# pytorch/audio

Hardware: NVIDIA H100
Metric: MelSpectrogram frames/sec (higher is better)
Workload: dtype f32

## Files before the change

audio_b200/csrc/frontend_pow2.cu:

```cuda
#include <type_traits>
#include <utility>

#include "common.cuh"
#include "f32x2.cuh"
#include "ptx.cuh"

namespace b200a {

namespace {

constexpr float kKaldiEps = 1.1920928955078125e-07f;
constexpr int kPadSymmetric = 4;
constexpr int kWarps = 8;
constexpr int kMelWarps = 4;
constexpr int kMaxItems = 64;
constexpr int kMaxItemsPerWarp = 32;
constexpr int kFragSmemSteps = 112;
constexpr int kMaxSlots = 64;

template <int G>
struct Geo {
  static constexpr int kNfft = 32 * G;
  static constexpr int kBins = kNfft / 2 + 1;
  static constexpr int kGroups = 32 / G;
  static constexpr int kFrames = 2 * kGroups;
  static constexpr int kRowLd = G + 1;
  static constexpr int kRegion = 32 * (G + 1) + (G == 8 ? 8 : 0);
  static constexpr int kTileF2 = kGroups * kRegion;
  static constexpr int kSlots = kWarps * kFrames;
  static constexpr int kPitch = ((kBins + 7 - 4 + 31) / 32) * 32 + 4;
  static constexpr int kLogG = G == 32 ? 5 : (G == 16 ? 4 : 3);
};

struct MelItem {
  int tile;
  int kstart;
  int nsteps;
  int frag_off;
};
struct MelPlan {
  int n_tiles, n_items, total_steps, pad;
  int warp_cnt[kWarps];
  int warp_items[kWarps][kMaxItemsPerWarp];
  MelItem items[kMaxItems];
};

struct Pow2Extra {
  size_t tw2d, tw_eo, plan, frags, total;
};

inline int mel_tiles(int n_mels) { return (n_mels + 7) / 8; }

inline Pow2Extra pow2_layout(const b200a_frontend_desc& d, size_t base) {
  Pow2Extra e{};
  const size_t n_bins = d.n_fft / 2 + 1;
  const size_t nt = d.n_mels > 0 ? mel_tiles(d.n_mels) : 0;
  size_t off = base;
  e.tw2d = off;
  off = align_up(off + sizeof(float2) * 32 * 32, 256);
  e.tw_eo = off;
  off = align_up(off + sizeof(float2) * 17 * 32, 256);
  e.plan = off;
  off = align_up(off + sizeof(MelPlan), 256);
  e.frags = off;
  off = align_up(off + sizeof(float4) * 32 * nt * ((n_bins + 7) / 8 + 1), 256);
  e.total = off;
  return e;
}

bool pow2_applicable(const b200a_frontend_desc& d) {
  return (d.n_fft == 2048 || d.n_fft == 1024 || d.n_fft == 512 || d.n_fft == 256) && d.onesided != 0;
}

template <int... Is, typename F>
__device__ __forceinline__ void static_for_impl(std::integer_sequence<int, Is...>, F&& f) {
  (f(std::integral_constant<int, Is>{}), ...);
}
template <int N, typename F>
__device__ __forceinline__ void static_for(F&& f) {
  static_for_impl(std::make_integer_sequence<int, N>{}, static_cast<F&&>(f));
}

__host__ __device__ constexpr int brev5(int v) {
  return ((v & 1) << 4) | ((v & 2) << 2) | (v & 4) | ((v & 8) >> 2) | ((v & 16) >> 4);
}
template <int LOG>
__host__ __device__ constexpr int brev(int v) {
  return brev5(v) >> (5 - LOG);
}

__device__ constexpr float kCos32[17] = {1.f, 0.98078528040323043f, 0.92387953251128674f, 0.83146961230254524f,
                                         0.70710678118654757f, 0.55557023301960229f, 0.38268343236508984f,
                                         0.19509032201612833f, 0.f, -0.19509032201612819f, -0.38268343236508973f,
                                         -0.55557023301960196f, -0.70710678118654746f, -0.83146961230254535f,
                                         -0.92387953251128674f, -0.98078528040323043f, -1.f};
__device__ constexpr float kSin32[17] = {0.f, 0.19509032201612825f, 0.38268343236508978f, 0.55557023301960218f,
                                         0.70710678118654746f, 0.83146961230254524f, 0.92387953251128674f,
                                         0.98078528040323043f, 1.f, 0.98078528040323043f, 0.92387953251128674f,
                                         0.83146961230254546f, 0.70710678118654757f, 0.55557023301960218f,
                                         0.38268343236508989f, 0.19509032201612861f, 0.f};

template <int E>
__device__ __forceinline__ void bfly(float2& a, float2& b) {
  if constexpr (E == 0) {
    const float2 t = b;
    b = sub2(a, t);
    a = add2(a, t);
  } else if constexpr (E == 8) {
    const float2 t = b;
    b = add_i(a, t);
    a = sub_i(a, t);
  } else if constexpr (E == 4) {
    constexpr float c = 0.70710678118654752f;
    const float2 t = sub_i(b, b);
    b = fmas2(-c, t, a);
    a = fmas2(c, t, a);
  } else if constexpr (E == 12) {
    constexpr float c = 0.70710678118654752f;
    const float2 u = add_i(b, b);
    b = fmas2(c, u, a);
    a = fmas2(-c, u, a);
  } else {
    constexpr float wr = kCos32[E], wi = -kSin32[E];
    const float2 p = cfma2(wr, wi, b, a);
    b = fma2(make_float2(2.f, 2.f), a, make_float2(-p.x, -p.y));
    a = p;
  }
}

template <int LEN, int OFF, int S0 = 0, int S1 = 5>
__device__ __forceinline__ void fft_regs(float2 (&a)[32]) {
  constexpr int kStages = LEN == 32 ? 5 : (LEN == 16 ? 4 : 3);
  constexpr int kFirst = S0, kLast = S1 < kStages ? S1 : kStages;
  static_for<kLast - kFirst>([&](auto si) {
    constexpr int len = 2 << (decltype(si)::value + kFirst);
    constexpr int half = len / 2;
    static_for<LEN / 2>([&](auto bi) {
      constexpr int b = decltype(bi)::value;
      constexpr int i = (b / half) * len, j = b % half;
      bfly<j*(32 / len)>(a[OFF + i + j], a[OFF + i + j + half]);
    });
  });
}

struct Pow2Params {
  const float* wave;
  int64_t length, row_stride, frames, units_per_row, total_units;
  float* out;
  float* group_max;
  int64_t rows_per_group;
  const float* window;
  const float2* tw2d;
  const MelPlan* plan;
  const float4* frags;
  const WsHeader* hdr;
  int hop, pad, center, pad_mode, n_mels;
  int stage, log_mels, bulk_ok, stage_ok;
  int out_width, out_col0, out_vec;
  int kaldi, k_off, k_win, k_dc, k_energy_mode, k_energy_col, k_log;
  float k_preemph, k_energy_floor;
  float power, db_mult, db_amin, db_offset;
};

__device__ __forceinline__ int frame_lead(const Pow2Params& p, int n_fft) {
  return p.kaldi ? p.k_off : (p.center ? n_fft / 2 : 0);
}

constexpr int kComplexOut = 3;

template <int POWER_MODE>
__device__ __forceinline__ float pow_of(float re, float im, float power) {
  if constexpr (POWER_MODE == 2) return fmaf(re, re, im * im);
  const float mag = hypotf(re, im);
  return power == 1.f ? mag : powf(mag, power);
}

struct GroupMax {
  float* dst;
  int64_t group;
  float value;
  __device__ __forceinline__ void flush() {
    if (dst == nullptr) return;
    const int64_t g0 = __shfl_sync(0xffffffffu, group, 0);
    if (__all_sync(0xffffffffu, group == g0)) {
      const float mx = warp_max(value);
      if ((threadIdx.x & 31) == 0 && g0 >= 0 && mx > -CUDART_INF_F) atomic_max_f32(dst + g0, mx);
    } else if (group >= 0 && value > -CUDART_INF_F) {
      atomic_max_f32(dst + group, value);
    }
    value = -CUDART_INF_F;
  }
  __device__ __forceinline__ void add(int64_t g, float v, bool valid) {
    if (dst == nullptr) return;
    if (!valid) {
      g = group;
      v = -CUDART_INF_F;
    }
    if (__any_sync(0xffffffffu, g != group && group >= 0)) flush();
    group = g;
    value = fmaxf(value, v);
  }
};

template <int N>
__device__ __forceinline__ void reg_alloc() {
  asm volatile("setmaxnreg.inc.sync.aligned.u32 %0;" ::"n"(N));
}
template <int N>
__device__ __forceinline__ void reg_dealloc() {
  asm volatile("setmaxnreg.dec.sync.aligned.u32 %0;" ::"n"(N));
}

struct UnitCursor {
  int64_t u, stride, step_rows, step_units, upr;
  int64_t row, ub, nrow, nub;
  __device__ __forceinline__ void init(int64_t first, int64_t stride_, int64_t units_per_row) {
    u = first;
    stride = stride_;
    upr = units_per_row;
    step_rows = stride / upr;
    step_units = stride - step_rows * upr;
    row = first / upr;
    ub = first - row * upr;
    nrow = row + step_rows;
    nub = ub + step_units;
    if (nub >= upr) { nub -= upr; ++nrow; }
  }
  __device__ __forceinline__ void advance() {
    u += stride;
    row = nrow;
    ub = nub;
    nrow += step_rows;
    nub += step_units;
    if (nub >= upr) { nub -= upr; ++nrow; }
  }
};

template <int G>
__device__ __forceinline__ bool bulk_eligible(const Pow2Params& p, int half, int64_t u, int64_t ub) {
  using Ge = Geo<G>;
  if (!p.bulk_ok || u >= p.total_units) return false;
  const int64_t t0 = ub * Ge::kFrames;
  const int64_t s0 = t0 * p.hop - half - p.pad;
  return t0 + Ge::kFrames <= p.frames && s0 >= 0 && s0 + (int64_t)(Ge::kFrames - 1) * p.hop + Ge::kNfft <= p.length;
}
template <int G>
__device__ __forceinline__ void issue_bulk(const Pow2Params& p, int half, int64_t row, int64_t ub, void* dst,
                                           uint64_t* bar) {
  using Ge = Geo<G>;
  const float* src = p.wave + row * p.row_stride + (ub * Ge::kFrames * p.hop - half - p.pad);
  const uint32_t bytes = (uint32_t)(Ge::kNfft + (Ge::kFrames - 1) * p.hop) * 4u;
  mbar_expect_tx(bar, bytes);
  bulk_g2s(dst, src, bytes, bar);
}

template <int POWER_MODE, int G, int HG, bool KALDI>
__device__ __forceinline__ void transform_unit(const Pow2Params& p, const float (&wreg)[32], const float2* s_tw,
                                               float2* tile, uint64_t* bar, uint32_t& parity, bool& staged,
                                               const UnitCursor& cur, int half, int lane, float (&pa)[17],
                                               float (&pb)[17]) {
  using Ge = Geo<G>;
  float* stage = reinterpret_cast<float*>(tile);
  const int gi = lane / G, l = lane % G;
  const int64_t row = cur.row, t0 = cur.ub * Ge::kFrames;
  const int64_t ta = t0 + 2 * gi, tb = ta + 1;
  const bool has_a = ta < p.frames, has_b = tb < p.frames;
  const float* __restrict__ x = p.wave + row * p.row_stride;
  const int64_t s0 = t0 * p.hop - half - p.pad;
  const int64_t sa = s0 + (int64_t)2 * gi * p.hop, sb = sa + p.hop;
  const bool next_staged = bulk_eligible<G>(p, half, cur.u + cur.stride, cur.nub);
  const int64_t last = p.frames - t0 < Ge::kFrames ? p.frames - t0 : Ge::kFrames;
  const bool interior = s0 >= 0 && s0 + (last - 1) * p.hop + Ge::kNfft <= p.length;

  float2 a[32];
  float2* grp_tile = tile + gi * Ge::kRegion;
  bool from_stage = staged;
  if (staged) {
    mbar_wait(bar, parity);
    parity ^= 1;
  } else if ((!interior || KALDI) && p.stage_ok) {
    const int span = Ge::kNfft + (Ge::kFrames - 1) * p.hop;
    const int len = (int)p.length, ext = len + 2 * p.pad, j0 = (int)(t0 * p.hop) - half, mode = p.pad_mode;
#pragma unroll 4
    for (int n = lane; n < span; n += 32) {
      int j = j0 + n;
      if ((unsigned)j >= (unsigned)ext) {
        if (mode == B200A_PAD_REFLECT)
          j = j < 0 ? -j : 2 * (ext - 1) - j;
        else if (mode == B200A_PAD_REPLICATE)
          j = j < 0 ? 0 : ext - 1;
        else if (mode == kPadSymmetric)
          j = j < 0 ? -1 - j : 2 * ext - 1 - j;
        else if (mode == B200A_PAD_CIRCULAR) {
          j %= ext;
          if (j < 0) j += ext;
        } else
          j = -1;
      }
      const int src = j - p.pad;
      if (j >= 0 && (unsigned)src < (unsigned)len)
        cp_async4(stage + n, x + src);
      else
        stage[n] = 0.f;
    }
    cp_async_wait_all();
    __syncwarp();
    from_stage = true;
  }
  if (KALDI && from_stage) {
    const float* fa = stage + 2 * gi * p.hop;
    const float* fb = fa + p.hop;
    const int win = p.k_win;
    float ma = 0.f, mb = 0.f;
    if (p.k_dc) {
#pragma unroll 4
      for (int n = l; n < win; n += G) {
        ma += fa[n];
        mb += fb[n];
      }
#pragma unroll
      for (int o = G / 2; o > 0; o >>= 1) {
        ma += __shfl_xor_sync(0xffffffffu, ma, o);
        mb += __shfl_xor_sync(0xffffffffu, mb, o);
      }
      ma /= (float)win;
      mb /= (float)win;
    }
    float ea = 0.f, eb = 0.f;
    if (p.k_energy_mode == 1) {
#pragma unroll 4
      for (int n = l; n < win; n += G) {
        const float da = fa[n] - ma, db = fb[n] - mb;
        ea = fmaf(da, da, ea);
        eb = fmaf(db, db, eb);
      }
    }
    const float c = p.k_preemph;
    static_for<32>([&](auto ji) {
      constexpr int j = decltype(ji)::value;
      const int n = l + G * j;
      float va = 0.f, vb = 0.f;
      if (n < win) {
        const int np = n > 0 ? n - 1 : 0;
        va = ((fa[n] - ma) - c * (fa[np] - ma)) * wreg[j];
        vb = ((fb[n] - mb) - c * (fb[np] - mb)) * wreg[j];
      }
      a[brev5(j)] = make_float2(va, vb);
      if (p.k_energy_mode == 2) {
        ea = fmaf(2.f * va, 2.f * va, ea);
        eb = fmaf(2.f * vb, 2.f * vb, eb);
      }
    });
    if (p.k_energy_mode != 0) {
#pragma unroll
      for (int o = G / 2; o > 0; o >>= 1) {
        ea += __shfl_xor_sync(0xffffffffu, ea, o);
        eb += __shfl_xor_sync(0xffffffffu, eb, o);
      }
      if (l == 0) {
        const float fl = p.k_energy_floor > 0.f ? logf(p.k_energy_floor) : -CUDART_INF_F;
        float* e_out = p.out + (row * p.frames + ta) * p.out_width + p.k_energy_col;
        if (has_a) e_out[0] = fmaxf(logf(fmaxf(ea, kKaldiEps)), fl);
        if (has_b) e_out[p.out_width] = fmaxf(logf(fmaxf(eb, kKaldiEps)), fl);
      }
    }
    __syncwarp();
  } else if (from_stage) {
    if constexpr (HG >= 0) {
      constexpr int kV = 32 + (HG >= 0 ? HG : 0);
      float v[kV];
      static_for<kV>([&](auto ji) {
        constexpr int j = decltype(ji)::value;
        v[j] = stage[lane + 32 * j];
      });
      static_for<32>([&](auto ji) {
        constexpr int j = decltype(ji)::value;
        a[brev5(j)] = make_float2(v[j] * wreg[j], v[j + (HG >= 0 ? HG : 0)] * wreg[j]);
      });
    } else {
      const float* pa_ptr = stage + 2 * gi * p.hop + l;
      const float* pb_ptr = pa_ptr + p.hop;
      static_for<32>([&](auto ji) {
        constexpr int j = decltype(ji)::value;
        a[brev5(j)] = scale2(wreg[j], make_float2(pa_ptr[G * j], pb_ptr[G * j]));
      });
    }
    __syncwarp();
  } else if (interior) {
    static_for<32>([&](auto ji) {
      constexpr int j = decltype(ji)::value;
      const float va = has_a ? __ldg(x + sa + l + G * j) : 0.f;
      const float vb = has_b ? __ldg(x + sb + l + G * j) : 0.f;
      a[brev5(j)] = scale2(wreg[j], make_float2(va, vb));
    });
  } else {
#pragma unroll 1
    for (int j = 0; j < 32; ++j) {
      const int n = l + G * j;
      const int64_t ia = has_a ? source_index(ta * p.hop + n, p.length, p.pad, half, p.pad_mode) : -1;
      const int64_t ib = has_b ? source_index(tb * p.hop + n, p.length, p.pad, half, p.pad_mode) : -1;
      grp_tile[n] = make_float2(ia >= 0 ? __ldg(x + ia) : 0.f, ib >= 0 ? __ldg(x + ib) : 0.f);
    }
    __syncwarp();
    static_for<32>([&](auto ji) {
      constexpr int j = decltype(ji)::value;
      const float2 v = grp_tile[l + G * j];
      a[brev5(j)] = scale2(wreg[j], v);
    });
    __syncwarp();
  }

  constexpr int kTwAhead = 8;
  fft_regs<32, 0, 0, 4>(a);
  float2 tw[32];
  static_for<kTwAhead>([&](auto ki) {
    constexpr int k2 = decltype(ki)::value + 1;
    tw[k2] = s_tw[k2 * G + l];
  });
  fft_regs<32, 0, 4, 5>(a);
  grp_tile[l] = a[0];
  static_for<31>([&](auto ki) {
    constexpr int k2 = decltype(ki)::value + 1;
    if constexpr (k2 + kTwAhead < 32) tw[k2 + kTwAhead] = s_tw[(k2 + kTwAhead) * G + l];
    grp_tile[k2 * Ge::kRowLd + l] = cmul2(a[k2], tw[k2]);
  });
  __syncwarp();
  static_for<32>([&](auto si) {
    constexpr int s = decltype(si)::value;
    constexpr int q = s / G, g = s % G;
    a[q * G + brev<Ge::kLogG>(g)] = grp_tile[(l + G * q) * Ge::kRowLd + g];
  });
  __syncwarp();
  staged = next_staged;
  if (staged && lane == 0) {
    asm volatile("fence.proxy.async.shared::cta;" ::: "memory");
    issue_bulk<G>(p, half, cur.nrow, cur.nub, stage, bar);
  }

  static_for<Ge::kGroups>([&](auto qi) { fft_regs<G, decltype(qi)::value * G>(a); });

  constexpr int NG = Ge::kGroups;
  const int src = (lane & ~(G - 1)) | ((G - l) & (G - 1));
  static_for<16>([&](auto mi) {
    constexpr int m = decltype(mi)::value;
    constexpr int slot = (m % NG) * G + m / NG;
    constexpr int mm = 31 - m, mslot = (mm % NG) * G + mm / NG;
    float mr = __shfl_sync(0xffffffffu, a[mslot].x, src);
    float mi_ = __shfl_sync(0xffffffffu, a[mslot].y, src);
    if (l == 0) {
      constexpr int m0 = (32 - m) & 31, slot0 = (m0 % NG) * G + m0 / NG;
      mr = a[slot0].x;
      mi_ = a[slot0].y;
    }
    const float zr = a[slot].x, zi = a[slot].y;
    const float2 sx = add2(make_float2(zr, zr), make_float2(mr, -mr));
    const float2 sy = add2(make_float2(zi, zi), make_float2(-mi_, mi_));
    if constexpr (POWER_MODE == kComplexOut) {
      float2* oc = reinterpret_cast<float2*>(p.out) + (row * p.frames + ta) * Ge::kBins + l + G * m;
      if (has_a) oc[0] = make_float2(sx.x, sy.x);
      if (has_b) oc[Ge::kBins] = make_float2(sy.y, -sx.y);
    } else if constexpr (POWER_MODE == 2) {
      const float2 pw = fma2(sx, sx, mul2(sy, sy));
      pa[m] = pw.x;
      pb[m] = pw.y;
    } else {
      pa[m] = pow_of<POWER_MODE>(sx.x, sy.x, p.power);
      pb[m] = pow_of<POWER_MODE>(sy.y, sx.y, p.power);
    }
  });
  constexpr int slot16 = (16 % NG) * G + 16 / NG;
  if constexpr (POWER_MODE == kComplexOut) {
    if (l == 0) {
      float2* oc = reinterpret_cast<float2*>(p.out) + (row * p.frames + ta) * Ge::kBins + Ge::kNfft / 2;
      if (has_a) oc[0] = make_float2(2.f * a[slot16].x, 0.f);
      if (has_b) oc[Ge::kBins] = make_float2(2.f * a[slot16].y, 0.f);
    }
  } else {
    pa[16] = pow_of<POWER_MODE>(2.f * a[slot16].x, 0.f, p.power);
    pb[16] = pow_of<POWER_MODE>(2.f * a[slot16].y, 0.f, p.power);
  }
}

template <int G>
__device__ __forceinline__ void load_window(const Pow2Params& p, int lane, float (&wreg)[32]) {
  const float hs = 0.5f * p.hdr->scale;
  const int l = lane % G;
#pragma unroll
  for (int j = 0; j < 32; ++j) wreg[j] = p.window[l + G * j] * hs;
}

template <int POWER_MODE, int G, int HG, int NW, bool KALDI>
__global__ void __launch_bounds__(NW * 32, 1) stft_pow2_power_kernel(const Pow2Params p) {
  using Ge = Geo<G>;
  extern __shared__ __align__(128) unsigned char smem_raw[];
  float2* s_tw = reinterpret_cast<float2*>(smem_raw);
  float2* s_tile_all = s_tw + 32 * 32;
  uint64_t* s_bar = reinterpret_cast<uint64_t*>(s_tile_all + NW * Ge::kTileF2);

  const int tid = threadIdx.x, lane = tid & 31, warp = tid >> 5;
  for (int i = tid; i < 32 * G; i += blockDim.x) s_tw[i] = p.tw2d[i];
  if (tid < NW) mbar_init(s_bar + tid, 1);
  asm volatile("fence.mbarrier_init.release.cluster;" ::: "memory");
  __syncthreads();

  float2* tile = s_tile_all + warp * Ge::kTileF2;
  float* stage = reinterpret_cast<float*>(tile);
  uint64_t* bar = s_bar + warp;
  float wreg[32];
  load_window<G>(p, lane, wreg);
  const int half = frame_lead(p, Ge::kNfft);
  const int gi = lane / G, l = lane % G;
  uint32_t parity = 0;
  bool staged = false;
  UnitCursor cur;
  cur.init((int64_t)blockIdx.x * NW + warp, (int64_t)gridDim.x * NW, p.units_per_row);
  if (bulk_eligible<G>(p, half, cur.u, cur.ub)) {
    if (lane == 0) issue_bulk<G>(p, half, cur.row, cur.ub, stage, bar);
    staged = true;
  }
  for (; cur.u < p.total_units; cur.advance()) {
    float pa[17], pb[17];
    transform_unit<POWER_MODE, G, HG, KALDI>(p, wreg, s_tw, tile, bar, parity, staged, cur, half, lane, pa, pb);
    if constexpr (POWER_MODE == kComplexOut) continue;
    const int64_t ta = cur.ub * Ge::kFrames + 2 * gi;
    const bool has_a = ta < p.frames, has_b = ta + 1 < p.frames;
    float* oa = p.out + (cur.row * p.frames + ta) * p.out_width + p.out_col0;
    float* ob = oa + p.out_width;
    if (KALDI && p.k_log) {
#pragma unroll
      for (int m = 0; m < 17; ++m) {
        pa[m] = logf(fmaxf(pa[m], kKaldiEps));
        pb[m] = logf(fmaxf(pb[m], kKaldiEps));
      }
    }
    const int skip = KALDI ? p.k_energy_col - p.out_col0 : -1;
#pragma unroll
    for (int m = 0; m < 16; ++m) {
      if (l + G * m == skip) continue;
      if (has_a) oa[l + G * m] = pa[m];
      if (has_b) ob[l + G * m] = pb[m];
    }
    if (l == 0 && Ge::kNfft / 2 != skip) {
      if (has_a) oa[Ge::kNfft / 2] = pa[16];
      if (has_b) ob[Ge::kNfft / 2] = pb[16];
    }
  }
}

template <int PITCH>
__device__ __forceinline__ void contract_tile(const Pow2Params& p, const MelPlan* s_plan, const float4* s_frags,
                                              bool frags_in_smem, int mw, int lane, const float* pw,
                                              const int64_t* slot, const int64_t* grp, GroupMax& gmax) {
  const int r = lane >> 2, c = lane & 3;
  const int cnt = s_plan->warp_cnt[mw];
  const int64_t o_lo = slot[r], o_hi = slot[r + 8];
  const int64_t g_lo = grp[r], g_hi = grp[r + 8];
  for (int ii = 0; ii < cnt; ++ii) {
    const MelItem mi = s_plan->items[s_plan->warp_items[mw][ii]];
    const float* a_lo_row = pw + (size_t)r * PITCH + mi.kstart + c;
    const float* a_hi_row = a_lo_row + 8 * PITCH;
    float d0[4] = {0.f, 0.f, 0.f, 0.f}, d1[4] = {0.f, 0.f, 0.f, 0.f}, d2[4] = {0.f, 0.f, 0.f, 0.f};
    auto contract = [&](auto in_smem) {
      const float4* fr = (decltype(in_smem)::value ? s_frags : p.frags) + (size_t)mi.frag_off * 32 + lane;
#pragma unroll 4
      for (int s = 0; s < mi.nsteps; ++s) {
        float4 bf;
        if constexpr (decltype(in_smem)::value) bf = fr[(size_t)s * 32];
        else bf = __ldg(fr + (size_t)s * 32);
        const float av[4] = {a_lo_row[8 * s], a_hi_row[8 * s], a_lo_row[8 * s + 4], a_hi_row[8 * s + 4]};
        uint32_t hi[4], lo[4];
#pragma unroll
        for (int q = 0; q < 4; ++q) split_tf32(av[q], hi[q], lo[q]);
        mma_tf32(d0, hi, __float_as_uint(bf.x), __float_as_uint(bf.y));
        mma_tf32(d1, lo, __float_as_uint(bf.x), __float_as_uint(bf.y));
        mma_tf32(d2, hi, __float_as_uint(bf.z), __float_as_uint(bf.w));
      }
    };
    if (frags_in_smem) contract(std::true_type{});
    else contract(std::false_type{});
    float d[4];
#pragma unroll
    for (int q = 0; q < 4; ++q) d[q] = d0[q] + (d1[q] + d2[q]);
    const int n0 = 8 * mi.tile + 2 * c;
    const bool n0_ok = n0 < p.n_mels, n1_ok = n0 + 1 < p.n_mels;
    if (p.k_log) {
#pragma unroll
      for (int q = 0; q < 4; ++q) d[q] = logf(fmaxf(d[q], kKaldiEps));
    }
    if (p.stage == B200A_STAGE_FEAT) {
#pragma unroll
      for (int q = 0; q < 4; ++q)
        d[q] = p.log_mels ? logf(d[q] + 1e-6f) : p.db_mult * log10f(fmaxf(d[q], p.db_amin)) - p.db_offset;
      const float m_lo = fmaxf(n0_ok ? d[0] : -CUDART_INF_F, n1_ok ? d[1] : -CUDART_INF_F);
      const float m_hi = fmaxf(n0_ok ? d[2] : -CUDART_INF_F, n1_ok ? d[3] : -CUDART_INF_F);
      gmax.add(g_lo, m_lo, o_lo >= 0);
      gmax.add(g_hi, m_hi, o_hi >= 0);
    }
    const bool vec = n1_ok && p.out_vec >= 2;
    if (o_lo >= 0) {
      if (vec) *reinterpret_cast<float2*>(p.out + o_lo + n0) = make_float2(d[0], d[1]);
      else {
        if (n0_ok) p.out[o_lo + n0] = d[0];
        if (n1_ok) p.out[o_lo + n0 + 1] = d[1];
      }
    }
    if (o_hi >= 0) {
      if (vec) *reinterpret_cast<float2*>(p.out + o_hi + n0) = make_float2(d[2], d[3]);
      else {
        if (n0_ok) p.out[o_hi + n0] = d[2];
        if (n1_ok) p.out[o_hi + n0 + 1] = d[3];
      }
    }
  }
}

constexpr int kFftRegs = 200, kMelRegs = 96;

template <int POWER_MODE, int G, int HG, int FFT_REGS, bool KALDI>
__device__ __forceinline__ void mel_body_mma(const Pow2Params& p, unsigned char* smem_raw) {
  using Ge = Geo<G>;
  constexpr int kSlots = Ge::kSlots, kPitch = Ge::kPitch;
  float2* s_tw = reinterpret_cast<float2*>(smem_raw);
  float2* s_tile_all = s_tw + 32 * 32;
  float* s_pow = reinterpret_cast<float*>(s_tile_all + kWarps * Ge::kTileF2);
  int64_t* s_slot = reinterpret_cast<int64_t*>(s_pow + 2 * kSlots * kPitch);
  int64_t* s_grp = s_slot + 2 * kSlots;
  uint64_t* s_bar = reinterpret_cast<uint64_t*>(s_grp + 2 * kSlots);
  uint64_t* s_full = s_bar + kWarps;
  uint64_t* s_empty = s_full + 2;
  MelPlan* s_plan = reinterpret_cast<MelPlan*>(s_empty + 2);
  float4* s_frags = reinterpret_cast<float4*>(s_plan + 1);

  const int tid = threadIdx.x, lane = tid & 31, warp = tid >> 5;
  for (int i = tid; i < 32 * G; i += blockDim.x) s_tw[i] = p.tw2d[i];
  {
    const int* src = reinterpret_cast<const int*>(p.plan);
    int* dst = reinterpret_cast<int*>(s_plan);
    for (int i = tid; i < (int)(sizeof(MelPlan) / sizeof(int)); i += blockDim.x) dst[i] = src[i];
  }
  const int total_steps = p.plan->total_steps;
  const bool frags_in_smem = total_steps <= kFragSmemSteps;
  if (frags_in_smem)
    for (int i = tid; i < total_steps * 32; i += blockDim.x) s_frags[i] = p.frags[i];
  for (int i = tid; i < 2 * kSlots * (kPitch - Ge::kBins); i += blockDim.x) {
    const int r = i / (kPitch - Ge::kBins), c = i - r * (kPitch - Ge::kBins);
    s_pow[r * kPitch + Ge::kBins + c] = 0.f;
  }
  if (tid < kWarps) mbar_init(s_bar + tid, 1);
  if (tid == 0) {
    mbar_init(s_full + 0, kWarps);
    mbar_init(s_full + 1, kWarps);
    mbar_init(s_empty + 0, kMelWarps);
    mbar_init(s_empty + 1, kMelWarps);
  }
  asm volatile("fence.mbarrier_init.release.cluster;" ::: "memory");
  __syncthreads();

  const int64_t stride = (int64_t)gridDim.x * kWarps;
  const int64_t u0 = (int64_t)blockIdx.x * kWarps;
  const int width = p.out_width;

  if (warp < kWarps) {
    reg_alloc<FFT_REGS>();
    float2* tile = s_tile_all + warp * Ge::kTileF2;
    float* stage = reinterpret_cast<float*>(tile);
    uint64_t* bar = s_bar + warp;
    float wreg[32];
    load_window<G>(p, lane, wreg);
    const int half = frame_lead(p, Ge::kNfft);
    const int gi = lane / G, l = lane % G;
    uint32_t parity = 0;
    bool staged = false;
    UnitCursor cur;
    cur.init(u0 + warp, stride, p.units_per_row);
    if (bulk_eligible<G>(p, half, cur.u, cur.ub)) {
      if (lane == 0) issue_bulk<G>(p, half, cur.row, cur.ub, stage, bar);
      staged = true;
    }
    int it = 0;
    for (int64_t base = u0; base < p.total_units; base += stride, ++it, cur.advance()) {
      const bool valid = cur.u < p.total_units;
      float pa[17], pb[17];
      if (valid)
        transform_unit<POWER_MODE, G, HG, KALDI>(p, wreg, s_tw, tile, bar, parity, staged, cur, half, lane, pa, pb);
      const int b = it & 1;
      if (it >= 2) mbar_wait(s_empty + b, ((it >> 1) & 1) ^ 1);
      const int slot_a = Ge::kFrames * warp + 2 * gi;
      float* prow_a = s_pow + (size_t)(b * kSlots + slot_a) * kPitch;
      float* prow_b = prow_a + kPitch;
      if (valid) {
#pragma unroll
        for (int m = 0; m < 16; ++m) {
          prow_a[l + G * m] = pa[m];
          prow_b[l + G * m] = pb[m];
        }
        if (l == 0) {
          prow_a[Ge::kNfft / 2] = pa[16];
          prow_b[Ge::kNfft / 2] = pb[16];
        }
      }
      if (l == 0) {
        const int64_t ta = cur.ub * Ge::kFrames + 2 * gi;
        const int64_t oa = (cur.row * p.frames + ta) * (int64_t)width + p.out_col0;
        s_slot[b * kSlots + slot_a] = (valid && ta < p.frames) ? oa : -1;
        s_slot[b * kSlots + slot_a + 1] = (valid && ta + 1 < p.frames) ? oa + width : -1;
        const int64_t g = cur.row / p.rows_per_group;
        s_grp[b * kSlots + slot_a] = g;
        s_grp[b * kSlots + slot_a + 1] = g;
      }
      __syncwarp();
      if (lane == 0) mbar_arrive(s_full + b);
    }
  } else {
    reg_dealloc<kMelRegs>();
    const int mw = warp - kWarps;
    GroupMax gmax{p.stage == B200A_STAGE_FEAT ? p.group_max : nullptr, -1, -CUDART_INF_F};
    int it = 0;
    for (int64_t base = u0; base < p.total_units; base += stride, ++it) {
      const int b = it & 1;
      mbar_wait(s_full + b, (it >> 1) & 1);
#pragma unroll 1
      for (int mt = 0; mt < kSlots / 16; ++mt)
        contract_tile<kPitch>(p, s_plan, s_frags, frags_in_smem, mw, lane, s_pow + (size_t)(b * kSlots + 16 * mt) * kPitch,
                              s_slot + b * kSlots + 16 * mt, s_grp + b * kSlots + 16 * mt, gmax);
      __syncwarp();
      if (lane == 0) mbar_arrive(s_empty + b);
    }
    gmax.flush();
  }
}

constexpr int kEoN = 2048, kEoBins = 1025, kEoPitch = 1060, kEoSlots = 16;
constexpr int kEoFragSteps = 136;

__device__ __forceinline__ bool eo_frame_bulk_ok(const Pow2Params& p, int half, int64_t t) {
  const int64_t sa = t * p.hop - half - p.pad;
  return p.bulk_ok && t < p.frames && sa >= 0 && sa + kEoN <= p.length;
}

template <int POWER_MODE>
__device__ __forceinline__ void transform_frame_eo(const Pow2Params& p, const float2* s_win, const float2* s_tw,
                                                   const float2* s_tw2, float2* tile, uint64_t* bar, uint32_t& parity,
                                                   bool& staged, int64_t row, int64_t t, bool next_ok, int64_t next_row,
                                                   int64_t next_t, int half, int lane, float (&plo)[16],
                                                   float (&phi)[16], float& pmid) {
  const float* __restrict__ x = p.wave + row * p.row_stride;
  const int64_t sa = t * p.hop - half - p.pad;
  float* stage = reinterpret_cast<float*>(tile);
  float2 a[32];
  if (staged) {
    mbar_wait(bar, parity);
    parity ^= 1;
    const float2* st2 = reinterpret_cast<const float2*>(stage);
    static_for<32>([&](auto ji) {
      constexpr int j = decltype(ji)::value;
      const float2 v = st2[lane + 32 * j], w = s_win[lane + 32 * j];
      a[brev5(j)] = make_float2(v.x * w.x, v.y * w.y);
    });
    __syncwarp();
  } else if (sa >= 0 && sa + kEoN <= p.length) {
    static_for<32>([&](auto ji) {
      constexpr int j = decltype(ji)::value;
      const float2 w = s_win[lane + 32 * j];
      const float ve = __ldg(x + sa + 2 * (lane + 32 * j)), vo = __ldg(x + sa + 2 * (lane + 32 * j) + 1);
      a[brev5(j)] = make_float2(ve * w.x, vo * w.y);
    });
  } else {
#pragma unroll 1
    for (int j = 0; j < 32; ++j) {
      const int m = lane + 32 * j;
      const int64_t ie = source_index(t * p.hop + 2 * m, p.length, p.pad, half, p.pad_mode);
      const int64_t io = source_index(t * p.hop + 2 * m + 1, p.length, p.pad, half, p.pad_mode);
      tile[m] = make_float2(ie >= 0 ? __ldg(x + ie) : 0.f, io >= 0 ? __ldg(x + io) : 0.f);
    }
    __syncwarp();
    static_for<32>([&](auto ji) {
      constexpr int j = decltype(ji)::value;
      const float2 v = tile[lane + 32 * j], w = s_win[lane + 32 * j];
      a[brev5(j)] = make_float2(v.x * w.x, v.y * w.y);
    });
    __syncwarp();
  }

  fft_regs<32, 0>(a);
  tile[lane] = a[0];
  static_for<31>([&](auto ki) {
    constexpr int k2 = decltype(ki)::value + 1;
    const float2 w = s_tw[k2 * 32 + lane];
    const float2 v = a[k2];
    tile[k2 * 33 + lane] = cmul2(v, w);
  });
  __syncwarp();
  static_for<32>([&](auto gi) {
    constexpr int g = decltype(gi)::value;
    a[brev5(g)] = tile[lane * 33 + g];
  });
  __syncwarp();
  staged = next_ok && eo_frame_bulk_ok(p, half, next_t);
  if (staged && lane == 0) {
    asm volatile("fence.proxy.async.shared::cta;" ::: "memory");
    const float* src = p.wave + next_row * p.row_stride + (next_t * p.hop - half - p.pad);
    mbar_expect_tx(bar, kEoN * 4u);
    bulk_g2s(stage, src, kEoN * 4u, bar);
  }
  fft_regs<32, 0>(a);

  const int src_lane = (32 - lane) & 31;
  static_for<16>([&](auto ki) {
    constexpr int k1 = decltype(ki)::value;
    float mr = __shfl_sync(0xffffffffu, a[31 - k1].x, src_lane);
    float mi = __shfl_sync(0xffffffffu, a[31 - k1].y, src_lane);
    if (lane == 0) {
      mr = a[(32 - k1) & 31].x;
      mi = a[(32 - k1) & 31].y;
    }
    const float zr = a[k1].x, zi = a[k1].y;
    const float er = zr + mr, ei = zi - mi;
    const float orr = zi + mi, oi = mr - zr;
    const float2 w = s_tw2[k1 * 32 + lane];
    const float tr = fmaf(orr, w.x, -oi * w.y), ti = fmaf(orr, w.y, oi * w.x);
    plo[k1] = pow_of<POWER_MODE>(er + tr, ei + ti, p.power);
    phi[k1] = pow_of<POWER_MODE>(er - tr, ei - ti, p.power);
  });
  pmid = pow_of<POWER_MODE>(2.f * a[16].x, -2.f * a[16].y, p.power);
}

__device__ __forceinline__ void eo_store_row(float* row, int lane, const float (&plo)[16], const float (&phi)[16],
                                             float pmid) {
#pragma unroll
  for (int k1 = 0; k1 < 16; ++k1) {
    row[lane + 32 * k1] = plo[k1];
    row[1024 - lane - 32 * k1] = phi[k1];
  }
  if (lane == 0) row[512] = pmid;
}

__device__ __forceinline__ void eo_load_tables(const Pow2Params& p, const float2* tw_eo, float2* s_win, float2* s_tw,
                                               float2* s_tw2, int tid, int nthreads) {
  const float hs = 0.5f * p.hdr->scale;
  for (int i = tid; i < 1024; i += nthreads) {
    s_tw[i] = p.tw2d[i];
    s_win[i] = make_float2(p.window[2 * i] * hs, p.window[2 * i + 1] * hs);
  }
  for (int i = tid; i < 17 * 32; i += nthreads) s_tw2[i] = tw_eo[i];
}

struct EoNext {
  bool ok;
  int64_t row, t;
};
__device__ __forceinline__ EoNext eo_next_frame(const Pow2Params& p, const UnitCursor& cur, int f) {
  if (f == 0) return EoNext{true, cur.row, 2 * cur.ub + 1};
  return EoNext{cur.u + cur.stride < p.total_units, cur.nrow, 2 * cur.nub};
}

template <int POWER_MODE>
__global__ void __launch_bounds__(kWarps * 32, 1) stft2048_power_kernel(const Pow2Params p, const float2* tw_eo) {
  extern __shared__ __align__(128) unsigned char smem_raw[];
  float2* s_tw = reinterpret_cast<float2*>(smem_raw);
  float2* s_win = s_tw + 1024;
  float2* s_tw2 = s_win + 1024;
  float2* s_tile_all = s_tw2 + 17 * 32;
  uint64_t* s_bar = reinterpret_cast<uint64_t*>(s_tile_all + kWarps * 32 * 33);
  const int tid = threadIdx.x, lane = tid & 31, warp = tid >> 5;
  eo_load_tables(p, tw_eo, s_win, s_tw, s_tw2, tid, blockDim.x);
  if (tid < kWarps) mbar_init(s_bar + tid, 1);
  asm volatile("fence.mbarrier_init.release.cluster;" ::: "memory");
  __syncthreads();
  float2* tile = s_tile_all + warp * 32 * 33;
  uint64_t* bar = s_bar + warp;
  const int half = p.center ? kEoN / 2 : 0;
  uint32_t parity = 0;
  bool staged = false;
  UnitCursor cur;
  cur.init((int64_t)blockIdx.x * kWarps + warp, (int64_t)gridDim.x * kWarps, p.units_per_row);
  if (cur.u < p.total_units && eo_frame_bulk_ok(p, half, 2 * cur.ub)) {
    if (lane == 0) {
      mbar_expect_tx(bar, kEoN * 4u);
      bulk_g2s(tile, p.wave + cur.row * p.row_stride + (2 * cur.ub * p.hop - half - p.pad), kEoN * 4u, bar);
    }
    staged = true;
  }
  for (; cur.u < p.total_units; cur.advance()) {
#pragma unroll 1
    for (int f = 0; f < 2; ++f) {
      const int64_t t = 2 * cur.ub + f;
      if (t >= p.frames) { staged = false; break; }
      const EoNext nx = eo_next_frame(p, cur, f);
      float plo[16], phi[16], pmid;
      transform_frame_eo<POWER_MODE>(p, s_win, s_tw, s_tw2, tile, bar, parity, staged, cur.row, t, nx.ok, nx.row, nx.t,
                                     half, lane, plo, phi, pmid);
      eo_store_row(p.out + (cur.row * p.frames + t) * kEoBins, lane, plo, phi, pmid);
    }
  }
}

template <int POWER_MODE>
__global__ void __launch_bounds__((kWarps + kMelWarps) * 32, 1) stft2048_mel_kernel(const Pow2Params p,
                                                                                     const float2* tw_eo) {
  extern __shared__ __align__(128) unsigned char smem_raw[];
  float2* s_tw = reinterpret_cast<float2*>(smem_raw);
  float2* s_win = s_tw + 1024;
  float2* s_tw2 = s_win + 1024;
  float2* s_tile_all = s_tw2 + 17 * 32;
  float* s_pow = reinterpret_cast<float*>(s_tile_all + kWarps * 32 * 33);
  int64_t* s_slot = reinterpret_cast<int64_t*>(s_pow + kEoSlots * kEoPitch);
  int64_t* s_grp = s_slot + kEoSlots;
  uint64_t* s_bar = reinterpret_cast<uint64_t*>(s_grp + kEoSlots);
  uint64_t* s_full = s_bar + kWarps;
  uint64_t* s_empty = s_full + 1;
  MelPlan* s_plan = reinterpret_cast<MelPlan*>(s_empty + 1);
  float4* s_frags = reinterpret_cast<float4*>(s_plan + 1);

  const int tid = threadIdx.x, lane = tid & 31, warp = tid >> 5;
  eo_load_tables(p, tw_eo, s_win, s_tw, s_tw2, tid, blockDim.x);
  {
    const int* src = reinterpret_cast<const int*>(p.plan);
    int* dst = reinterpret_cast<int*>(s_plan);
    for (int i = tid; i < (int)(sizeof(MelPlan) / sizeof(int)); i += blockDim.x) dst[i] = src[i];
  }
  const int total_steps = p.plan->total_steps;
  const bool frags_in_smem = total_steps <= kEoFragSteps;
  if (frags_in_smem)
    for (int i = tid; i < total_steps * 32; i += blockDim.x) s_frags[i] = p.frags[i];
  for (int i = tid; i < kEoSlots * (kEoPitch - kEoBins); i += blockDim.x) {
    const int r = i / (kEoPitch - kEoBins), c = i - r * (kEoPitch - kEoBins);
    s_pow[r * kEoPitch + kEoBins + c] = 0.f;
  }
  if (tid < kWarps) mbar_init(s_bar + tid, 1);
  if (tid == 0) {
    mbar_init(s_full, kWarps);
    mbar_init(s_empty, kMelWarps);
  }
  asm volatile("fence.mbarrier_init.release.cluster;" ::: "memory");
  __syncthreads();

  const int64_t stride = (int64_t)gridDim.x * kWarps;
  const int64_t u0 = (int64_t)blockIdx.x * kWarps;
  if (warp < kWarps) {
    reg_alloc<kFftRegs>();
    float2* tile = s_tile_all + warp * 32 * 33;
    uint64_t* bar = s_bar + warp;
    const int half = p.center ? kEoN / 2 : 0;
    uint32_t parity = 0;
    bool staged = false;
    UnitCursor cur;
    cur.init(u0 + warp, stride, p.units_per_row);
    if (cur.u < p.total_units && eo_frame_bulk_ok(p, half, 2 * cur.ub)) {
      if (lane == 0) {
        mbar_expect_tx(bar, kEoN * 4u);
        bulk_g2s(tile, p.wave + cur.row * p.row_stride + (2 * cur.ub * p.hop - half - p.pad), kEoN * 4u, bar);
      }
      staged = true;
    }
    int it = 0;
    for (int64_t base = u0; base < p.total_units; base += stride, ++it, cur.advance()) {
      const bool valid = cur.u < p.total_units;
#pragma unroll 1
      for (int f = 0; f < 2; ++f) {
        const int64_t t = 2 * cur.ub + f;
        const bool live = valid && t < p.frames;
        float plo[16], phi[16], pmid = 0.f;
        if (live) {
          const EoNext nx = eo_next_frame(p, cur, f);
          transform_frame_eo<POWER_MODE>(p, s_win, s_tw, s_tw2, tile, bar, parity, staged, cur.row, t, nx.ok, nx.row,
                                         nx.t, half, lane, plo, phi, pmid);
        } else {
          staged = false;
        }
        if (f == 0 && it >= 1) mbar_wait(s_empty, (it - 1) & 1);
        if (live) eo_store_row(s_pow + (size_t)(2 * warp + f) * kEoPitch, lane, plo, phi, pmid);
        if (lane == 0) {
          s_slot[2 * warp + f] = live ? (cur.row * p.frames + t) * (int64_t)p.n_mels : -1;
          s_grp[2 * warp + f] = cur.row / p.rows_per_group;
        }
      }
      __syncwarp();
      if (lane == 0) mbar_arrive(s_full);
    }
  } else {
    reg_dealloc<kMelRegs>();
    const int mw = warp - kWarps;
    GroupMax gmax{p.stage == B200A_STAGE_FEAT ? p.group_max : nullptr, -1, -CUDART_INF_F};
    int it = 0;
    for (int64_t base = u0; base < p.total_units; base += stride, ++it) {
      mbar_wait(s_full, it & 1);
      contract_tile<kEoPitch>(p, s_plan, s_frags, frags_in_smem, mw, lane, s_pow, s_slot, s_grp, gmax);
      __syncwarp();
      if (lane == 0) mbar_arrive(s_empty);
    }
    gmax.flush();
  }
}

__global__ void prepare_tw_eo_kernel(float2* tw_eo) {
  const int i = blockIdx.x * blockDim.x + threadIdx.x;
  if (i < 17 * 32) {
    const int k1 = i >> 5, l = i & 31;
    double s, c;
    sincospi(-2.0 * (double)(l + 32 * k1) / 2048.0, &s, &c);
    tw_eo[i] = make_float2((float)c, (float)s);
  }
}

template <int POWER_MODE, int G, int HG, bool KALDI>
__global__ void __launch_bounds__((kWarps + kMelWarps) * 32, 1) stft_pow2_mel_kernel(const Pow2Params p) {
  extern __shared__ __align__(128) unsigned char smem_raw[];
  mel_body_mma<POWER_MODE, G, HG, kFftRegs, KALDI>(p, smem_raw);
}

struct IstftPow2Params {
  const float2* spec;
  int64_t stride_row, stride_bin, stride_frame;
  int64_t frames, units_per_row, total_units;
  float* frame_buf;
  const float* window;
  const float2* tw2d;
  const WsHeader* hdr;
};

constexpr int kIsWarps = 16;

template <int G>
__global__ void __launch_bounds__(kIsWarps * 32, 1) istft_pow2_kernel(const IstftPow2Params p) {
  using Ge = Geo<G>;
  constexpr int N = Ge::kNfft, NG = Ge::kGroups;
  extern __shared__ __align__(128) unsigned char smem_raw[];
  float2* s_tw = reinterpret_cast<float2*>(smem_raw);
  float2* s_tile_all = s_tw + 32 * G;
  const int tid = threadIdx.x, lane = tid & 31, warp = tid >> 5;
  for (int i = tid; i < 32 * G; i += blockDim.x) s_tw[i] = p.tw2d[i];
  __syncthreads();
  float2* grp_tile = s_tile_all + warp * Ge::kTileF2 + (lane / G) * Ge::kRegion;
  const int gi = lane / G, l = lane % G;
  float wreg[32];
  {
    const float gain = 1.f / ((float)N * p.hdr->scale);
#pragma unroll
    for (int m = 0; m < 32; ++m) wreg[m] = p.window[l + G * m] * gain;
  }
  UnitCursor cur;
  cur.init((int64_t)blockIdx.x * kIsWarps + warp, (int64_t)gridDim.x * kIsWarps, p.units_per_row);
  for (; cur.u < p.total_units; cur.advance()) {
    const int64_t ta = cur.ub * Ge::kFrames + 2 * gi, tb = ta + 1;
    const bool has_a = ta < p.frames, has_b = tb < p.frames;
    const float2* __restrict__ sp = p.spec + cur.row * p.stride_row;
    float2 a[32];
    static_for<32>([&](auto ji) {
      constexpr int j = decltype(ji)::value;
      const int n = l + G * j;
      const int kk = n <= N / 2 ? n : N - n;
      float2 za = make_float2(0.f, 0.f), zb = za;
      if (has_a) za = __ldg(sp + kk * p.stride_bin + ta * p.stride_frame);
      if (has_b) zb = __ldg(sp + kk * p.stride_bin + tb * p.stride_frame);
      if (kk == 0 || kk == N / 2) za.y = zb.y = 0.f;
      if (n > N / 2) {
        za.y = -za.y;
        zb.y = -zb.y;
      }
      a[brev5(j)] = make_float2(za.x - zb.y, -(za.y + zb.x));
    });
    fft_regs<32, 0>(a);
    grp_tile[l] = a[0];
    static_for<31>([&](auto ki) {
      constexpr int k2 = decltype(ki)::value + 1;
      const float2 w = s_tw[k2 * G + l];
      const float2 v = a[k2];
      grp_tile[k2 * Ge::kRowLd + l] = cmul2(v, w);
    });
    __syncwarp();
    static_for<32>([&](auto si) {
      constexpr int s = decltype(si)::value;
      constexpr int q = s / G, g = s % G;
      a[q * G + brev<Ge::kLogG>(g)] = grp_tile[(l + G * q) * Ge::kRowLd + g];
    });
    __syncwarp();
    static_for<NG>([&](auto qi) { fft_regs<G, decltype(qi)::value * G>(a); });
    float* fa = p.frame_buf + (cur.row * p.frames + ta) * N + l;
    static_for<32>([&](auto mi) {
      constexpr int m = decltype(mi)::value;
      constexpr int slot = (m % NG) * G + m / NG;
      if (has_a) fa[G * m] = a[slot].x * wreg[m];
      if (has_b) fa[N + G * m] = -a[slot].y * wreg[m];
    });
  }
}

__global__ void prepare_tw2d_kernel(float2* tw2d, int G) {
  const int i = blockIdx.x * blockDim.x + threadIdx.x;
  if (i < 32 * G) {
    const int k2 = i / G, g = i - k2 * G;
    double s, c;
    sincospi(-2.0 * (double)(k2 * g) / (double)(32 * G), &s, &c);
    tw2d[i] = make_float2((float)c, (float)s);
  }
}

__global__ void prepare_mma_kernel(const float* __restrict__ fb, const int2* __restrict__ bands, int n_bins, int n_mels,
                                   int n_tiles, MelPlan* plan, float4* frags) {
  __shared__ int t_kstart[kMaxItems], t_steps[kMaxItems];
  if (threadIdx.x == 0) {
    int total = 0;
    for (int t = 0; t < n_tiles; ++t) {
      int lo = n_bins, hi = 0;
      for (int m = 8 * t; m < min(8 * t + 8, n_mels); ++m) {
        const int2 b = bands[m];
        if (b.y > b.x) { lo = min(lo, b.x); hi = max(hi, b.y); }
      }
      t_kstart[t] = hi > lo ? (lo & ~7) : 0;
      t_steps[t] = hi > lo ? (hi - t_kstart[t] + 7) / 8 : 0;
      plan->items[t] = MelItem{t, t_kstart[t], t_steps[t], total};
      total += t_steps[t];
    }
    plan->n_tiles = n_tiles;
    plan->n_items = n_tiles;
    plan->total_steps = total;
    plan->pad = 0;
    int load[kWarps];
    bool used[kMaxItems];
    for (int w = 0; w < kWarps; ++w) { load[w] = 0; plan->warp_cnt[w] = 0; }
    for (int i = 0; i < n_tiles; ++i) used[i] = false;
    for (int k = 0; k < n_tiles; ++k) {
      int best = -1;
      for (int i = 0; i < n_tiles; ++i)
        if (!used[i] && (best < 0 || t_steps[i] > t_steps[best])) best = i;
      used[best] = true;
      int w = 0;
      for (int q = 1; q < kMelWarps; ++q)
        if (load[q] < load[w] || (load[q] == load[w] && plan->warp_cnt[q] < plan->warp_cnt[w])) w = q;
      plan->warp_items[w][plan->warp_cnt[w]++] = best;
      load[w] += t_steps[best] + 2;
    }
  }
  __syncthreads();
  int off = 0;
  for (int t = 0; t < n_tiles; ++t) {
    for (int i = threadIdx.x; i < t_steps[t] * 32; i += blockDim.x) {
      const int s = i >> 5, lane = i & 31;
      const int n = 8 * t + (lane >> 2);
      const int k0 = t_kstart[t] + 8 * s + (lane & 3), k1 = k0 + 4;
      const float b0 = (n < n_mels && k0 < n_bins) ? fb[(size_t)k0 * n_mels + n] : 0.f;
      const float b1 = (n < n_mels && k1 < n_bins) ? fb[(size_t)k1 * n_mels + n] : 0.f;
      const float b0h = __uint_as_float(__float_as_uint(b0) & 0xffffe000u);
      const float b1h = __uint_as_float(__float_as_uint(b1) & 0xffffe000u);
      frags[(size_t)(off + s) * 32 + lane] = make_float4(b0h, b1h, b0 - b0h, b1 - b1h);
    }
    off += t_steps[t];
  }
}

static_assert(kMaxItemsPerWarp * kMelWarps >= kMaxItems,
              "every filter group must find a place in a contraction warp's list");

}

size_t pow2_workspace_extra(const b200a_frontend_desc* d) {
  if (!pow2_applicable(*d)) return 0;
  const size_t base = ws_layout(*d).total;
  return pow2_layout(*d, base).total - base;
}

int pow2_prepare(const b200a_frontend_desc* d, void* ws, size_t ws_bytes, cudaStream_t stream) {
  if (!pow2_applicable(*d)) return B200A_OK;
  const WsLayout l = ws_layout(*d);
  const Pow2Extra e = pow2_layout(*d, l.total);
  if (ws_bytes < e.total) return B200A_EWORKSPACE;
  unsigned char* base = static_cast<unsigned char*>(ws);
  const int G = d->n_fft == 2048 ? 32 : d->n_fft / 32;
  prepare_tw2d_kernel<<<(32 * G + 255) / 256, 256, 0, stream>>>(reinterpret_cast<float2*>(base + e.tw2d), G);
  if (d->n_fft == 2048) prepare_tw_eo_kernel<<<3, 256, 0, stream>>>(reinterpret_cast<float2*>(base + e.tw_eo));
  if (d->n_mels > 0 && mel_tiles(d->n_mels) <= kMaxItems) {
    prepare_mma_kernel<<<1, 256, 0, stream>>>(reinterpret_cast<const float*>(base + l.fb),
                                              reinterpret_cast<const int2*>(base + l.bands), d->n_fft / 2 + 1, d->n_mels,
                                              mel_tiles(d->n_mels), reinterpret_cast<MelPlan*>(base + e.plan),
                                              reinterpret_cast<float4*>(base + e.frags));
  }
  return launch_status();
}

static int num_sms() { return device_sm_count(); }

static int64_t persistent_grid(const Pow2Params& p, int warps = kWarps) {
  const int sms = num_sms();
  if (sms < 0) return -1;
  const int64_t iters = (p.total_units + warps - 1) / warps;
  const int64_t grid = iters < sms ? iters : sms;
  return grid < 1 ? 1 : grid;
}

template <int POWER_MODE, int G, int HG>
static int launch_power(const Pow2Params& p, cudaStream_t stream) {
  using Ge = Geo<G>;
  constexpr int NW = 16;
  const size_t smem = sizeof(float2) * (32 * 32 + NW * Ge::kTileF2) + sizeof(uint64_t) * NW;
  auto kern = stft_pow2_power_kernel<POWER_MODE, G, HG, NW, false>;
  if constexpr (POWER_MODE != kComplexOut)
    if (p.kaldi) kern = stft_pow2_power_kernel<POWER_MODE, G, -1, NW, true>;
  if (cudaFuncSetAttribute(kern, cudaFuncAttributeMaxDynamicSharedMemorySize, 227 * 1024) != cudaSuccess)
    return B200A_ECUDA;
  const int64_t grid = persistent_grid(p, NW);
  if (grid < 0) return B200A_ECUDA;
  kern<<<(unsigned)grid, NW * 32, smem, stream>>>(p);
  return launch_status();
}

template <int POWER_MODE, int G, int HG>
static int launch_mel(const Pow2Params& p, cudaStream_t stream) {
  using Ge = Geo<G>;
  static_assert(sizeof(MelPlan) % 16 == 0, "fragment array must stay 16-byte aligned");
  static_assert(Ge::kSlots <= kMaxSlots, "slot tables");
  const size_t smem = sizeof(float2) * (32 * 32 + kWarps * Ge::kTileF2) + sizeof(float) * 2 * Ge::kSlots * Ge::kPitch +
                      sizeof(int64_t) * 4 * Ge::kSlots + sizeof(uint64_t) * (kWarps + 4) + sizeof(MelPlan) +
                      sizeof(float4) * 32 * kFragSmemSteps;
  if (smem > 227 * 1024) return B200A_EUNSUPPORTED;
  auto kern = p.kaldi ? stft_pow2_mel_kernel<POWER_MODE, G, -1, true> : stft_pow2_mel_kernel<POWER_MODE, G, HG, false>;
  if (cudaFuncSetAttribute(kern, cudaFuncAttributeMaxDynamicSharedMemorySize, 227 * 1024) != cudaSuccess)
    return B200A_ECUDA;
  const int64_t grid = persistent_grid(p);
  if (grid < 0) return B200A_ECUDA;
  kern<<<(unsigned)grid, (kWarps + kMelWarps) * 32, smem, stream>>>(p);
  return launch_status();
}

template <int POWER_MODE, int G>
static int launch_g(const Pow2Params& p, bool mel, cudaStream_t stream) {
  if constexpr (POWER_MODE == kComplexOut) {
    if constexpr (G == 32)
      if (p.bulk_ok && p.hop == 256) return launch_power<POWER_MODE, 32, 8>(p, stream);
    return launch_power<POWER_MODE, G, -1>(p, stream);
  } else {
    if constexpr (G == 32) {
      if (p.bulk_ok && p.hop == 256 && !p.kaldi)
        return mel ? launch_mel<POWER_MODE, 32, 8>(p, stream) : launch_power<POWER_MODE, 32, 8>(p, stream);
    }
    return mel ? launch_mel<POWER_MODE, G, -1>(p, stream) : launch_power<POWER_MODE, G, -1>(p, stream);
  }
}

template <int POWER_MODE>
static int launch_any(Pow2Params& p, int n_fft, bool mel, cudaStream_t stream) {
  if (n_fft == 1024) return launch_g<POWER_MODE, 32>(p, mel, stream);
  if (n_fft == 512) return launch_g<POWER_MODE, 16>(p, mel, stream);
  return launch_g<POWER_MODE, 8>(p, mel, stream);
}

template <int POWER_MODE>
static int launch_eo(const Pow2Params& p, const float2* tw_eo, bool mel, cudaStream_t stream) {
  const int64_t grid = persistent_grid(p);
  if (grid < 0) return B200A_ECUDA;
  const size_t tables = sizeof(float2) * (1024 + 1024 + 17 * 32 + kWarps * 32 * 33);
  if (!mel) {
    auto kern = stft2048_power_kernel<POWER_MODE>;
    if (cudaFuncSetAttribute(kern, cudaFuncAttributeMaxDynamicSharedMemorySize, 227 * 1024) != cudaSuccess)
      return B200A_ECUDA;
    kern<<<(unsigned)grid, kWarps * 32, tables + sizeof(uint64_t) * kWarps, stream>>>(p, tw_eo);
    return launch_status();
  }
  const size_t smem = tables + sizeof(float) * kEoSlots * kEoPitch + sizeof(int64_t) * 2 * kEoSlots +
                      sizeof(uint64_t) * (kWarps + 2) + sizeof(MelPlan) + sizeof(float4) * 32 * kEoFragSteps;
  if (smem > 227 * 1024) return B200A_EUNSUPPORTED;
  auto kern = stft2048_mel_kernel<POWER_MODE>;
  if (cudaFuncSetAttribute(kern, cudaFuncAttributeMaxDynamicSharedMemorySize, 227 * 1024) != cudaSuccess)
    return B200A_ECUDA;
  kern<<<(unsigned)grid, (kWarps + kMelWarps) * 32, smem, stream>>>(p, tw_eo);
  return launch_status();
}

int frontend_run_pow2(const b200a_frontend_desc* d, const void* ws, int stage, const float* wave, int64_t rows,
                      int64_t length, int64_t row_stride, int64_t frames, float* out, float* group_max,
                      int64_t rows_per_group, cudaStream_t stream, const b200a_kaldi_desc* kd) {
  if (!pow2_applicable(*d)) return B200A_EUNSUPPORTED;
  if (stage == B200A_STAGE_COMPLEX && (d->n_fft > 1024 || kd != nullptr)) return B200A_EUNSUPPORTED;
  if (kd != nullptr && d->n_fft > 1024) return B200A_EUNSUPPORTED;
  if (stage >= B200A_STAGE_MEL && mel_tiles(d->n_mels) > kMaxItems) return B200A_EUNSUPPORTED;
  const WsLayout l = ws_layout(*d);
  const Pow2Extra e = pow2_layout(*d, l.total);
  const unsigned char* base = static_cast<const unsigned char*>(ws);
  const bool eo = d->n_fft == 2048;
  const int G = eo ? 32 : d->n_fft / 32;
  const int frames_per_unit = 2 * (32 / G);
  Pow2Params p{};
  p.wave = wave;
  p.length = length;
  p.row_stride = row_stride;
  p.frames = frames;
  p.units_per_row = (frames + frames_per_unit - 1) / frames_per_unit;
  p.total_units = rows * p.units_per_row;
  p.out = out;
  p.group_max = group_max;
  p.rows_per_group = rows_per_group > 0 ? rows_per_group : 1;
  p.window = reinterpret_cast<const float*>(base + l.window);
  p.tw2d = reinterpret_cast<const float2*>(base + e.tw2d);
  p.plan = reinterpret_cast<const MelPlan*>(base + e.plan);
  p.frags = reinterpret_cast<const float4*>(base + e.frags);
  p.hdr = reinterpret_cast<const WsHeader*>(base + l.header);
  p.hop = d->hop;
  p.pad = d->pad;
  p.center = d->center;
  p.pad_mode = d->pad_mode;
  p.n_mels = d->n_mels;
  p.stage = stage;
  p.log_mels = d->log_mels;
  p.power = d->power;
  p.db_mult = d->db_multiplier;
  p.db_amin = d->db_amin;
  p.db_offset = d->db_offset;
  const int half = d->center ? d->n_fft / 2 : 0;
  const int stage_floats = 2 * (32 / G) * (32 * (G + 1) + (G == 8 ? 8 : 0));
  p.bulk_ok = d->hop % 4 == 0 && (half + d->pad) % 4 == 0 && row_stride % 4 == 0 &&
              (reinterpret_cast<uintptr_t>(wave) & 15) == 0 &&
              d->n_fft + (frames_per_unit - 1) * (int64_t)d->hop <= stage_floats;
  p.stage_ok = d->n_fft + (frames_per_unit - 1) * (int64_t)d->hop <= stage_floats &&
               length + 2 * (int64_t)d->pad + d->n_fft < (int64_t)1 << 31;
  p.out_width = stage >= B200A_STAGE_MEL ? d->n_mels : d->n_fft / 2 + 1;
  p.out_col0 = 0;
  p.k_energy_col = -1;
  int lead = half;
  if (kd != nullptr) {
    p.kaldi = 1;
    p.k_off = kd->snip_edges ? 0 : kd->window_size / 2 - kd->window_shift / 2;
    p.k_win = kd->window_size;
    p.k_dc = kd->remove_dc_offset;
    p.k_preemph = kd->preemphasis;
    p.k_energy_mode = kd->energy_col >= 0 ? kd->energy_mode : 0;
    p.k_energy_floor = kd->energy_floor;
    p.k_energy_col = kd->energy_col;
    p.k_log = kd->use_log;
    p.out_width = kd->out_width;
    p.out_col0 = kd->out_col0;
    p.pad_mode = kPadSymmetric;
    lead = p.k_off;
    if (!p.stage_ok) return B200A_EUNSUPPORTED;
    p.bulk_ok = d->hop % 4 == 0 && lead % 4 == 0 && row_stride % 4 == 0 && (reinterpret_cast<uintptr_t>(wave) & 15) == 0;
  }
  p.out_vec = (p.out_width % 4 == 0 && p.out_col0 % 4 == 0 && (reinterpret_cast<uintptr_t>(out) & 15) == 0)   ? 4
              : (p.out_width % 2 == 0 && p.out_col0 % 2 == 0 && (reinterpret_cast<uintptr_t>(out) & 7) == 0) ? 2
                                                                                                              : 1;
  const bool mel = stage >= B200A_STAGE_MEL;
  if (eo) {
    p.bulk_ok = d->hop % 4 == 0 && (half + d->pad) % 4 == 0 && row_stride % 4 == 0 &&
                (reinterpret_cast<uintptr_t>(wave) & 15) == 0;
    const float2* tw_eo = reinterpret_cast<const float2*>(base + e.tw_eo);
    return d->power == 2.f ? launch_eo<2>(p, tw_eo, mel, stream) : launch_eo<0>(p, tw_eo, mel, stream);
  }
  if (stage == B200A_STAGE_COMPLEX) return launch_any<kComplexOut>(p, d->n_fft, false, stream);
  return d->power == 2.f ? launch_any<2>(p, d->n_fft, mel, stream) : launch_any<0>(p, d->n_fft, mel, stream);
}

int istft_frames_pow2(const b200a_frontend_desc* d, const void* ws, const float* spec, int64_t rows, int64_t frames,
                      int64_t stride_row, int64_t stride_bin, int64_t stride_frame, float* frame_buf, cudaStream_t stream) {
  if (!pow2_applicable(*d) || d->n_fft > 1024) return B200A_EUNSUPPORTED;
  const WsLayout l = ws_layout(*d);
  const Pow2Extra e = pow2_layout(*d, l.total);
  const unsigned char* base = static_cast<const unsigned char*>(ws);
  const int G = d->n_fft / 32;
  const int frames_per_unit = 2 * (32 / G);
  IstftPow2Params p{};
  p.spec = reinterpret_cast<const float2*>(spec);
  p.stride_row = stride_row;
  p.stride_bin = stride_bin;
  p.stride_frame = stride_frame;
  p.frames = frames;
  p.units_per_row = (frames + frames_per_unit - 1) / frames_per_unit;
  p.total_units = rows * p.units_per_row;
  p.frame_buf = frame_buf;
  p.window = reinterpret_cast<const float*>(base + l.window);
  p.tw2d = reinterpret_cast<const float2*>(base + e.tw2d);
  p.hdr = reinterpret_cast<const WsHeader*>(base + l.header);
  const int sms = num_sms();
  if (sms < 0) return B200A_ECUDA;
  const int64_t iters = (p.total_units + kIsWarps - 1) / kIsWarps;
  const unsigned grid = (unsigned)(iters < sms ? (iters < 1 ? 1 : iters) : sms);
  auto launch = [&](auto kern, size_t smem) {
    if (cudaFuncSetAttribute(kern, cudaFuncAttributeMaxDynamicSharedMemorySize, 227 * 1024) != cudaSuccess) return (int)B200A_ECUDA;
    kern<<<grid, kIsWarps * 32, smem, stream>>>(p);
    return launch_status();
  };
  if (G == 32) return launch(istft_pow2_kernel<32>, sizeof(float2) * (32 * 32 + kIsWarps * Geo<32>::kTileF2));
  if (G == 16) return launch(istft_pow2_kernel<16>, sizeof(float2) * (32 * 16 + kIsWarps * Geo<16>::kTileF2));
  return launch(istft_pow2_kernel<8>, sizeof(float2) * (32 * 8 + kIsWarps * Geo<8>::kTileF2));
}

}
```

Measured before the change: 521.4 million.

## Unify mel kernel into 16 uniform warps with split FFT transpose and smem window

Restructures the mel spectrogram kernel from 8 FFT warps plus 4 MMA warps into 16 uniform warps. Each warp does both the FFT and the tensor-core mel contraction, with a new per-warp work list of (m-tile, mel-tile) items built in the prepare kernel. The window moves from 32 per-thread registers into shared memory. A SPLIT mode does the FFT transpose through a float-only region, real and imaginary halves in turn, to shrink the per-warp shared-memory footprint. The aim is to cut register pressure and idle producer/consumer warps, at the cost of extra shared-memory traffic and syncwarps in the transpose.

New measurement: 568.2 million, median of 6. 1.09x the previous value.

```diff
diff --git a/audio_b200/csrc/frontend_pow2.cu b/audio_b200/csrc/frontend_pow2.cu
--- a/audio_b200/csrc/frontend_pow2.cu
+++ b/audio_b200/csrc/frontend_pow2.cu
@@ -13,10 +13,13 @@
 constexpr int kPadSymmetric = 4;
 constexpr int kWarps = 8;
 constexpr int kMelWarps = 4;
+constexpr int kUniWarps = 16;
 constexpr int kMaxItems = 64;
 constexpr int kMaxItemsPerWarp = 32;
+constexpr int kMaxMTiles = 8;
 constexpr int kFragSmemSteps = 112;
-constexpr int kMaxSlots = 64;
+constexpr int kMaxSlots = 128;
+constexpr int kSmemLimit = 227 * 1024;
 
 template <int G>
 struct Geo {
@@ -27,9 +30,14 @@
   static constexpr int kRowLd = G + 1;
   static constexpr int kRegion = 32 * (G + 1) + (G == 8 ? 8 : 0);
   static constexpr int kTileF2 = kGroups * kRegion;
-  static constexpr int kSlots = kWarps * kFrames;
-  static constexpr int kPitch = ((kBins + 7 - 4 + 31) / 32) * 32 + 4;
+  static constexpr int kRegionF = 32 * (G + 1) + (G < 32 ? G : 0);
+  static constexpr int kMelRegion = G == 32 ? 1536 : (G == 16 ? 1504 : 1472);
+  static constexpr int kMelFragSteps = G == 32 ? 100 : kFragSmemSteps;
+  static constexpr int kSlots = kUniWarps * kFrames;
+  static constexpr int kMTiles = kSlots / 16;
+  static constexpr int kPitch = (kBins + 7) / 8 * 8 + 4;
   static constexpr int kLogG = G == 32 ? 5 : (G == 16 ? 4 : 3);
+  static_assert(kMelRegion >= kGroups * kRegionF && kMelRegion % 4 == 0, "mel warp region");
 };
 
 struct MelItem {
@@ -39,9 +47,11 @@
   int frag_off;
 };
 struct MelPlan {
-  int n_tiles, n_items, total_steps, pad;
-  int warp_cnt[kWarps];
-  int warp_items[kWarps][kMaxItemsPerWarp];
+  int n_tiles, n_items, total_steps, n_work;
+  int warp_cnt[kMelWarps];
+  int warp_items[kMelWarps][kMaxItemsPerWarp];
+  int work_begin[kUniWarps + 4];
+  unsigned short work[kMaxMTiles * kMaxItems];
   MelItem items[kMaxItems];
 };
 
@@ -254,8 +264,8 @@
   bulk_g2s(dst, src, bytes, bar);
 }
 
-template <int POWER_MODE, int G, int HG, bool KALDI>
-__device__ __forceinline__ void transform_unit(const Pow2Params& p, const float (&wreg)[32], const float2* s_tw,
+template <int POWER_MODE, int G, int HG, bool KALDI, bool SPLIT>
+__device__ __forceinline__ void transform_unit(const Pow2Params& p, const float* s_win, const float2* s_tw,
                                                float2* tile, uint64_t* bar, uint32_t& parity, bool& staged,
                                                const UnitCursor& cur, int half, int lane, float (&pa)[17],
                                                float (&pb)[17]) {
@@ -274,6 +284,7 @@
 
   float2 a[32];
   float2* grp_tile = tile + gi * Ge::kRegion;
+  float* grp_f = stage + gi * (SPLIT ? Ge::kRegionF : 2 * Ge::kRegion);
   bool from_stage = staged;
   if (staged) {
     mbar_wait(bar, parity);
@@ -342,8 +353,9 @@
       float va = 0.f, vb = 0.f;
       if (n < win) {
         const int np = n > 0 ? n - 1 : 0;
-        va = ((fa[n] - ma) - c * (fa[np] - ma)) * wreg[j];
-        vb = ((fb[n] - mb) - c * (fb[np] - mb)) * wreg[j];
+        const float w = s_win[n];
+        va = ((fa[n] - ma) - c * (fa[np] - ma)) * w;
+        vb = ((fb[n] - mb) - c * (fb[np] - mb)) * w;
       }
       a[brev5(j)] = make_float2(va, vb);
       if (p.k_energy_mode == 2) {
@@ -375,14 +387,15 @@
       });
       static_for<32>([&](auto ji) {
         constexpr int j = decltype(ji)::value;
-        a[brev5(j)] = make_float2(v[j] * wreg[j], v[j + (HG >= 0 ? HG : 0)] * wreg[j]);
+        const float w = s_win[lane + 32 * j];
+        a[brev5(j)] = make_float2(v[j] * w, v[j + (HG >= 0 ? HG : 0)] * w);
       });
     } else {
       const float* pa_ptr = stage + 2 * gi * p.hop + l;
       const float* pb_ptr = pa_ptr + p.hop;
       static_for<32>([&](auto ji) {
         constexpr int j = decltype(ji)::value;
-        a[brev5(j)] = scale2(wreg[j], make_float2(pa_ptr[G * j], pb_ptr[G * j]));
+        a[brev5(j)] = scale2(s_win[l + G * j], make_float2(pa_ptr[G * j], pb_ptr[G * j]));
       });
     }
     __syncwarp();
@@ -391,23 +404,27 @@
       constexpr int j = decltype(ji)::value;
       const float va = has_a ? __ldg(x + sa + l + G * j) : 0.f;
       const float vb = has_b ? __ldg(x + sb + l + G * j) : 0.f;
-      a[brev5(j)] = scale2(wreg[j], make_float2(va, vb));
+      a[brev5(j)] = scale2(s_win[l + G * j], make_float2(va, vb));
     });
   } else {
+#pragma unroll
+    for (int f = 0; f < 2; ++f) {
+      const int64_t t = ta + f;
 #pragma unroll 1
-    for (int j = 0; j < 32; ++j) {
-      const int n = l + G * j;
-      const int64_t ia = has_a ? source_index(ta * p.hop + n, p.length, p.pad, half, p.pad_mode) : -1;
-      const int64_t ib = has_b ? source_index(tb * p.hop + n, p.length, p.pad, half, p.pad_mode) : -1;
-      grp_tile[n] = make_float2(ia >= 0 ? __ldg(x + ia) : 0.f, ib >= 0 ? __ldg(x + ib) : 0.f);
-    }
-    __syncwarp();
-    static_for<32>([&](auto ji) {
-      constexpr int j = decltype(ji)::value;
-      const float2 v = grp_tile[l + G * j];
-      a[brev5(j)] = scale2(wreg[j], v);
-    });
-    __syncwarp();
+      for (int j = 0; j < 32; ++j) {
+        const int n = l + G * j;
+        const int64_t i = t < p.frames ? source_index(t * p.hop + n, p.length, p.pad, half, p.pad_mode) : -1;
+        grp_f[n] = i >= 0 ? __ldg(x + i) : 0.f;
+      }
+      __syncwarp();
+      static_for<32>([&](auto ji) {
+        constexpr int j = decltype(ji)::value;
+        const float v = __fmul_rn(s_win[l + G * j], grp_f[l + G * j]);
+        if (f == 0) a[brev5(j)].x = v;
+        else a[brev5(j)].y = v;
+      });
+      __syncwarp();
+    }
   }
 
   constexpr int kTwAhead = 8;
@@ -418,18 +435,45 @@
     tw[k2] = s_tw[k2 * G + l];
   });
   fft_regs<32, 0, 4, 5>(a);
-  grp_tile[l] = a[0];
-  static_for<31>([&](auto ki) {
-    constexpr int k2 = decltype(ki)::value + 1;
-    if constexpr (k2 + kTwAhead < 32) tw[k2 + kTwAhead] = s_tw[(k2 + kTwAhead) * G + l];
-    grp_tile[k2 * Ge::kRowLd + l] = cmul2(a[k2], tw[k2]);
-  });
-  __syncwarp();
-  static_for<32>([&](auto si) {
-    constexpr int s = decltype(si)::value;
-    constexpr int q = s / G, g = s % G;
-    a[q * G + brev<Ge::kLogG>(g)] = grp_tile[(l + G * q) * Ge::kRowLd + g];
-  });
+  if constexpr (SPLIT) {
+    grp_f[l] = a[0].x;
+    static_for<31>([&](auto ki) {
+      constexpr int k2 = decltype(ki)::value + 1;
+      if constexpr (k2 + kTwAhead < 32) tw[k2 + kTwAhead] = s_tw[(k2 + kTwAhead) * G + l];
+      a[k2] = cmul2(a[k2], tw[k2]);
+      grp_f[k2 * Ge::kRowLd + l] = a[k2].x;
+    });
+    __syncwarp();
+    float re[32];
+    static_for<32>([&](auto si) {
+      constexpr int s = decltype(si)::value;
+      re[s] = grp_f[(l + G * (s / G)) * Ge::kRowLd + s % G];
+    });
+    __syncwarp();
+    static_for<32>([&](auto ki) {
+      constexpr int k2 = decltype(ki)::value;
+      grp_f[k2 * Ge::kRowLd + l] = a[k2].y;
+    });
+    __syncwarp();
+    static_for<32>([&](auto si) {
+      constexpr int s = decltype(si)::value;
+      constexpr int q = s / G, g = s % G;
+      a[q * G + brev<Ge::kLogG>(g)] = make_float2(re[s], grp_f[(l + G * q) * Ge::kRowLd + g]);
+    });
+  } else {
+    grp_tile[l] = a[0];
+    static_for<31>([&](auto ki) {
+      constexpr int k2 = decltype(ki)::value + 1;
+      if constexpr (k2 + kTwAhead < 32) tw[k2 + kTwAhead] = s_tw[(k2 + kTwAhead) * G + l];
+      grp_tile[k2 * Ge::kRowLd + l] = cmul2(a[k2], tw[k2]);
+    });
+    __syncwarp();
+    static_for<32>([&](auto si) {
+      constexpr int s = decltype(si)::value;
+      constexpr int q = s / G, g = s % G;
+      a[q * G + brev<Ge::kLogG>(g)] = grp_tile[(l + G * q) * Ge::kRowLd + g];
+    });
+  }
   __syncwarp();
   staged = next_staged;
   if (staged && lane == 0) {
@@ -481,12 +525,9 @@
   }
 }
 
-template <int G>
-__device__ __forceinline__ void load_window(const Pow2Params& p, int lane, float (&wreg)[32]) {
+__device__ __forceinline__ void load_window(const Pow2Params& p, float* s_win, int n, int tid, int nthreads) {
   const float hs = 0.5f * p.hdr->scale;
-  const int l = lane % G;
-#pragma unroll
-  for (int j = 0; j < 32; ++j) wreg[j] = p.window[l + G * j] * hs;
+  for (int i = tid; i < n; i += nthreads) s_win[i] = p.window[i] * hs;
 }
 
 template <int POWER_MODE, int G, int HG, int NW, bool KALDI>
@@ -494,11 +535,13 @@
   using Ge = Geo<G>;
   extern __shared__ __align__(128) unsigned char smem_raw[];
   float2* s_tw = reinterpret_cast<float2*>(smem_raw);
-  float2* s_tile_all = s_tw + 32 * 32;
+  float* s_win = reinterpret_cast<float*>(s_tw + 32 * 32);
+  float2* s_tile_all = reinterpret_cast<float2*>(s_win + Ge::kNfft);
   uint64_t* s_bar = reinterpret_cast<uint64_t*>(s_tile_all + NW * Ge::kTileF2);
 
   const int tid = threadIdx.x, lane = tid & 31, warp = tid >> 5;
   for (int i = tid; i < 32 * G; i += blockDim.x) s_tw[i] = p.tw2d[i];
+  load_window(p, s_win, Ge::kNfft, tid, blockDim.x);
   if (tid < NW) mbar_init(s_bar + tid, 1);
   asm volatile("fence.mbarrier_init.release.cluster;" ::: "memory");
   __syncthreads();
@@ -506,8 +549,6 @@
   float2* tile = s_tile_all + warp * Ge::kTileF2;
   float* stage = reinterpret_cast<float*>(tile);
   uint64_t* bar = s_bar + warp;
-  float wreg[32];
-  load_window<G>(p, lane, wreg);
   const int half = frame_lead(p, Ge::kNfft);
   const int gi = lane / G, l = lane % G;
   uint32_t parity = 0;
@@ -520,7 +561,7 @@
   }
   for (; cur.u < p.total_units; cur.advance()) {
     float pa[17], pb[17];
-    transform_unit<POWER_MODE, G, HG, KALDI>(p, wreg, s_tw, tile, bar, parity, staged, cur, half, lane, pa, pb);
+    transform_unit<POWER_MODE, G, HG, KALDI, false>(p, s_win, s_tw, tile, bar, parity, staged, cur, half, lane, pa, pb);
     if constexpr (POWER_MODE == kComplexOut) continue;
     const int64_t ta = cur.ub * Ge::kFrames + 2 * gi;
     const bool has_a = ta < p.frames, has_b = ta + 1 < p.frames;
@@ -548,186 +589,182 @@
 }
 
 template <int PITCH>
+__device__ __forceinline__ void contract_item(const Pow2Params& p, const MelItem& mi, const float4* s_frags,
+                                              bool frags_in_smem, int lane, const float* pw, int64_t o_lo,
+                                              int64_t o_hi, int64_t g_lo, int64_t g_hi, GroupMax& gmax) {
+  const int r = lane >> 2, c = lane & 3;
+  const float* a_lo_row = pw + (size_t)r * PITCH + mi.kstart + c;
+  const float* a_hi_row = a_lo_row + 8 * PITCH;
+  float d0[4] = {0.f, 0.f, 0.f, 0.f}, d1[4] = {0.f, 0.f, 0.f, 0.f}, d2[4] = {0.f, 0.f, 0.f, 0.f};
+  auto contract = [&](auto in_smem) {
+    const float4* fr = (decltype(in_smem)::value ? s_frags : p.frags) + (size_t)mi.frag_off * 32 + lane;
+#pragma unroll 4
+    for (int s = 0; s < mi.nsteps; ++s) {
+      float4 bf;
+      if constexpr (decltype(in_smem)::value) bf = fr[(size_t)s * 32];
+      else bf = __ldg(fr + (size_t)s * 32);
+      const float av[4] = {a_lo_row[8 * s], a_hi_row[8 * s], a_lo_row[8 * s + 4], a_hi_row[8 * s + 4]};
+      uint32_t hi[4], lo[4];
+#pragma unroll
+      for (int q = 0; q < 4; ++q) split_tf32(av[q], hi[q], lo[q]);
+      mma_tf32(d0, hi, __float_as_uint(bf.x), __float_as_uint(bf.y));
+      mma_tf32(d1, lo, __float_as_uint(bf.x), __float_as_uint(bf.y));
+      mma_tf32(d2, hi, __float_as_uint(bf.z), __float_as_uint(bf.w));
+    }
+  };
+  if (frags_in_smem) contract(std::true_type{});
+  else contract(std::false_type{});
+  float d[4];
+#pragma unroll
+  for (int q = 0; q < 4; ++q) d[q] = d0[q] + (d1[q] + d2[q]);
+  const int n0 = 8 * mi.tile + 2 * c;
+  const bool n0_ok = n0 < p.n_mels, n1_ok = n0 + 1 < p.n_mels;
+  if (p.k_log) {
+#pragma unroll
+    for (int q = 0; q < 4; ++q) d[q] = logf(fmaxf(d[q], kKaldiEps));
+  }
+  if (p.stage == B200A_STAGE_FEAT) {
+#pragma unroll
+    for (int q = 0; q < 4; ++q)
+      d[q] = p.log_mels ? logf(d[q] + 1e-6f) : p.db_mult * log10f(fmaxf(d[q], p.db_amin)) - p.db_offset;
+    const float m_lo = fmaxf(n0_ok ? d[0] : -CUDART_INF_F, n1_ok ? d[1] : -CUDART_INF_F);
+    const float m_hi = fmaxf(n0_ok ? d[2] : -CUDART_INF_F, n1_ok ? d[3] : -CUDART_INF_F);
+    gmax.add(g_lo, m_lo, o_lo >= 0);
+    gmax.add(g_hi, m_hi, o_hi >= 0);
+  }
+  const bool vec = n1_ok && p.out_vec >= 2;
+  if (o_lo >= 0) {
+    if (vec) *reinterpret_cast<float2*>(p.out + o_lo + n0) = make_float2(d[0], d[1]);
+    else {
+      if (n0_ok) p.out[o_lo + n0] = d[0];
+      if (n1_ok) p.out[o_lo + n0 + 1] = d[1];
+    }
+  }
+  if (o_hi >= 0) {
+    if (vec) *reinterpret_cast<float2*>(p.out + o_hi + n0) = make_float2(d[2], d[3]);
+    else {
+      if (n0_ok) p.out[o_hi + n0] = d[2];
+      if (n1_ok) p.out[o_hi + n0 + 1] = d[3];
+    }
+  }
+}
+
+template <int PITCH>
 __device__ __forceinline__ void contract_tile(const Pow2Params& p, const MelPlan* s_plan, const float4* s_frags,
                                               bool frags_in_smem, int mw, int lane, const float* pw,
                                               const int64_t* slot, const int64_t* grp, GroupMax& gmax) {
-  const int r = lane >> 2, c = lane & 3;
+  const int r = lane >> 2;
   const int cnt = s_plan->warp_cnt[mw];
   const int64_t o_lo = slot[r], o_hi = slot[r + 8];
   const int64_t g_lo = grp[r], g_hi = grp[r + 8];
-  for (int ii = 0; ii < cnt; ++ii) {
-    const MelItem mi = s_plan->items[s_plan->warp_items[mw][ii]];
-    const float* a_lo_row = pw + (size_t)r * PITCH + mi.kstart + c;
-    const float* a_hi_row = a_lo_row + 8 * PITCH;
-    float d0[4] = {0.f, 0.f, 0.f, 0.f}, d1[4] = {0.f, 0.f, 0.f, 0.f}, d2[4] = {0.f, 0.f, 0.f, 0.f};
-    auto contract = [&](auto in_smem) {
-      const float4* fr = (decltype(in_smem)::value ? s_frags : p.frags) + (size_t)mi.frag_off * 32 + lane;
-#pragma unroll 4
-      for (int s = 0; s < mi.nsteps; ++s) {
-        float4 bf;
-        if constexpr (decltype(in_smem)::value) bf = fr[(size_t)s * 32];
-        else bf = __ldg(fr + (size_t)s * 32);
-        const float av[4] = {a_lo_row[8 * s], a_hi_row[8 * s], a_lo_row[8 * s + 4], a_hi_row[8 * s + 4]};
-        uint32_t hi[4], lo[4];
-#pragma unroll
-        for (int q = 0; q < 4; ++q) split_tf32(av[q], hi[q], lo[q]);
-        mma_tf32(d0, hi, __float_as_uint(bf.x), __float_as_uint(bf.y));
-        mma_tf32(d1, lo, __float_as_uint(bf.x), __float_as_uint(bf.y));
-        mma_tf32(d2, hi, __float_as_uint(bf.z), __float_as_uint(bf.w));
-      }
-    };
-    if (frags_in_smem) contract(std::true_type{});
-    else contract(std::false_type{});
-    float d[4];
-#pragma unroll
-    for (int q = 0; q < 4; ++q) d[q] = d0[q] + (d1[q] + d2[q]);
-    const int n0 = 8 * mi.tile + 2 * c;
-    const bool n0_ok = n0 < p.n_mels, n1_ok = n0 + 1 < p.n_mels;
-    if (p.k_log) {
-#pragma unroll
-      for (int q = 0; q < 4; ++q) d[q] = logf(fmaxf(d[q], kKaldiEps));
-    }
-    if (p.stage == B200A_STAGE_FEAT) {
-#pragma unroll
-      for (int q = 0; q < 4; ++q)
-        d[q] = p.log_mels ? logf(d[q] + 1e-6f) : p.db_mult * log10f(fmaxf(d[q], p.db_amin)) - p.db_offset;
-      const float m_lo = fmaxf(n0_ok ? d[0] : -CUDART_INF_F, n1_ok ? d[1] : -CUDART_INF_F);
-      const float m_hi = fmaxf(n0_ok ? d[2] : -CUDART_INF_F, n1_ok ? d[3] : -CUDART_INF_F);
-      gmax.add(g_lo, m_lo, o_lo >= 0);
-      gmax.add(g_hi, m_hi, o_hi >= 0);
-    }
-    const bool vec = n1_ok && p.out_vec >= 2;
-    if (o_lo >= 0) {
-      if (vec) *reinterpret_cast<float2*>(p.out + o_lo + n0) = make_float2(d[0], d[1]);
-      else {
-        if (n0_ok) p.out[o_lo + n0] = d[0];
-        if (n1_ok) p.out[o_lo + n0 + 1] = d[1];
-      }
-    }
-    if (o_hi >= 0) {
-      if (vec) *reinterpret_cast<float2*>(p.out + o_hi + n0) = make_float2(d[2], d[3]);
-      else {
-        if (n0_ok) p.out[o_hi + n0] = d[2];
-        if (n1_ok) p.out[o_hi + n0 + 1] = d[3];
-      }
-    }
-  }
+  for (int ii = 0; ii < cnt; ++ii)
+    contract_item<PITCH>(p, s_plan->items[s_plan->warp_items[mw][ii]], s_frags, frags_in_smem, lane, pw, o_lo, o_hi,
+                         g_lo, g_hi, gmax);
 }
 
 constexpr int kFftRegs = 200, kMelRegs = 96;
 
-template <int POWER_MODE, int G, int HG, int FFT_REGS, bool KALDI>
-__device__ __forceinline__ void mel_body_mma(const Pow2Params& p, unsigned char* smem_raw) {
+template <int G>
+constexpr size_t mel_smem_bytes() {
+  using Ge = Geo<G>;
+  return sizeof(float2) * 32 * G + sizeof(float) * Ge::kNfft + sizeof(float) * kUniWarps * Ge::kMelRegion +
+         sizeof(float) * Ge::kSlots * Ge::kPitch + sizeof(int64_t) * 2 * Ge::kSlots + sizeof(uint64_t) * kUniWarps +
+         sizeof(MelPlan) + sizeof(float4) * 32 * Ge::kMelFragSteps;
+}
+
+template <int POWER_MODE, int G, int HG, bool KALDI>
+__device__ __forceinline__ void mel_body(const Pow2Params& p, unsigned char* smem_raw) {
   using Ge = Geo<G>;
   constexpr int kSlots = Ge::kSlots, kPitch = Ge::kPitch;
   float2* s_tw = reinterpret_cast<float2*>(smem_raw);
-  float2* s_tile_all = s_tw + 32 * 32;
-  float* s_pow = reinterpret_cast<float*>(s_tile_all + kWarps * Ge::kTileF2);
-  int64_t* s_slot = reinterpret_cast<int64_t*>(s_pow + 2 * kSlots * kPitch);
-  int64_t* s_grp = s_slot + 2 * kSlots;
-  uint64_t* s_bar = reinterpret_cast<uint64_t*>(s_grp + 2 * kSlots);
-  uint64_t* s_full = s_bar + kWarps;
-  uint64_t* s_empty = s_full + 2;
-  MelPlan* s_plan = reinterpret_cast<MelPlan*>(s_empty + 2);
+  float* s_win = reinterpret_cast<float*>(s_tw + 32 * G);
+  float* s_region_all = s_win + Ge::kNfft;
+  float* s_pow = s_region_all + kUniWarps * Ge::kMelRegion;
+  int64_t* s_slot = reinterpret_cast<int64_t*>(s_pow + kSlots * kPitch);
+  int64_t* s_grp = s_slot + kSlots;
+  uint64_t* s_bar = reinterpret_cast<uint64_t*>(s_grp + kSlots);
+  MelPlan* s_plan = reinterpret_cast<MelPlan*>(s_bar + kUniWarps);
   float4* s_frags = reinterpret_cast<float4*>(s_plan + 1);
 
   const int tid = threadIdx.x, lane = tid & 31, warp = tid >> 5;
   for (int i = tid; i < 32 * G; i += blockDim.x) s_tw[i] = p.tw2d[i];
+  load_window(p, s_win, Ge::kNfft, tid, blockDim.x);
   {
     const int* src = reinterpret_cast<const int*>(p.plan);
     int* dst = reinterpret_cast<int*>(s_plan);
     for (int i = tid; i < (int)(sizeof(MelPlan) / sizeof(int)); i += blockDim.x) dst[i] = src[i];
   }
   const int total_steps = p.plan->total_steps;
-  const bool frags_in_smem = total_steps <= kFragSmemSteps;
+  const bool frags_in_smem = total_steps <= Ge::kMelFragSteps;
   if (frags_in_smem)
     for (int i = tid; i < total_steps * 32; i += blockDim.x) s_frags[i] = p.frags[i];
-  for (int i = tid; i < 2 * kSlots * (kPitch - Ge::kBins); i += blockDim.x) {
+  for (int i = tid; i < kSlots * (kPitch - Ge::kBins); i += blockDim.x) {
     const int r = i / (kPitch - Ge::kBins), c = i - r * (kPitch - Ge::kBins);
     s_pow[r * kPitch + Ge::kBins + c] = 0.f;
   }
-  if (tid < kWarps) mbar_init(s_bar + tid, 1);
-  if (tid == 0) {
-    mbar_init(s_full + 0, kWarps);
-    mbar_init(s_full + 1, kWarps);
-    mbar_init(s_empty + 0, kMelWarps);
-    mbar_init(s_empty + 1, kMelWarps);
-  }
+  if (tid < kUniWarps) mbar_init(s_bar + tid, 1);
   asm volatile("fence.mbarrier_init.release.cluster;" ::: "memory");
   __syncthreads();
 
-  const int64_t stride = (int64_t)gridDim.x * kWarps;
-  const int64_t u0 = (int64_t)blockIdx.x * kWarps;
+  const int64_t stride = (int64_t)gridDim.x * kUniWarps;
+  const int64_t u0 = (int64_t)blockIdx.x * kUniWarps;
   const int width = p.out_width;
-
-  if (warp < kWarps) {
-    reg_alloc<FFT_REGS>();
-    float2* tile = s_tile_all + warp * Ge::kTileF2;
-    float* stage = reinterpret_cast<float*>(tile);
-    uint64_t* bar = s_bar + warp;
-    float wreg[32];
-    load_window<G>(p, lane, wreg);
-    const int half = frame_lead(p, Ge::kNfft);
-    const int gi = lane / G, l = lane % G;
-    uint32_t parity = 0;
-    bool staged = false;
-    UnitCursor cur;
-    cur.init(u0 + warp, stride, p.units_per_row);
-    if (bulk_eligible<G>(p, half, cur.u, cur.ub)) {
-      if (lane == 0) issue_bulk<G>(p, half, cur.row, cur.ub, stage, bar);
-      staged = true;
-    }
-    int it = 0;
-    for (int64_t base = u0; base < p.total_units; base += stride, ++it, cur.advance()) {
-      const bool valid = cur.u < p.total_units;
-      float pa[17], pb[17];
-      if (valid)
-        transform_unit<POWER_MODE, G, HG, KALDI>(p, wreg, s_tw, tile, bar, parity, staged, cur, half, lane, pa, pb);
-      const int b = it & 1;
-      if (it >= 2) mbar_wait(s_empty + b, ((it >> 1) & 1) ^ 1);
-      const int slot_a = Ge::kFrames * warp + 2 * gi;
-      float* prow_a = s_pow + (size_t)(b * kSlots + slot_a) * kPitch;
-      float* prow_b = prow_a + kPitch;
-      if (valid) {
+  float2* tile = reinterpret_cast<float2*>(s_region_all + warp * Ge::kMelRegion);
+  float* stage = reinterpret_cast<float*>(tile);
+  uint64_t* bar = s_bar + warp;
+  const int half = frame_lead(p, Ge::kNfft);
+  const int gi = lane / G, l = lane % G;
+  const int work_begin = s_plan->work_begin[warp], work_end = s_plan->work_begin[warp + 1];
+  GroupMax gmax{p.stage == B200A_STAGE_FEAT ? p.group_max : nullptr, -1, -CUDART_INF_F};
+  uint32_t parity = 0;
+  bool staged = false;
+  UnitCursor cur;
+  cur.init(u0 + warp, stride, p.units_per_row);
+  if (bulk_eligible<G>(p, half, cur.u, cur.ub)) {
+    if (lane == 0) issue_bulk<G>(p, half, cur.row, cur.ub, stage, bar);
+    staged = true;
+  }
+  for (int64_t base = u0; base < p.total_units; base += stride, cur.advance()) {
+    const bool valid = cur.u < p.total_units;
+    float pa[17], pb[17];
+    if (valid)
+      transform_unit<POWER_MODE, G, HG, KALDI, true>(p, s_win, s_tw, tile, bar, parity, staged, cur, half, lane, pa, pb);
+    __syncthreads();
+    const int slot_a = Ge::kFrames * warp + 2 * gi;
+    float* prow_a = s_pow + (size_t)slot_a * kPitch;
+    float* prow_b = prow_a + kPitch;
+    if (valid) {
 #pragma unroll
-        for (int m = 0; m < 16; ++m) {
-          prow_a[l + G * m] = pa[m];
-          prow_b[l + G * m] = pb[m];
-        }
-        if (l == 0) {
-          prow_a[Ge::kNfft / 2] = pa[16];
-          prow_b[Ge::kNfft / 2] = pb[16];
-        }
+      for (int m = 0; m < 16; ++m) {
+        prow_a[l + G * m] = pa[m];
+        prow_b[l + G * m] = pb[m];
       }
       if (l == 0) {
-        const int64_t ta = cur.ub * Ge::kFrames + 2 * gi;
-        const int64_t oa = (cur.row * p.frames + ta) * (int64_t)width + p.out_col0;
-        s_slot[b * kSlots + slot_a] = (valid && ta < p.frames) ? oa : -1;
-        s_slot[b * kSlots + slot_a + 1] = (valid && ta + 1 < p.frames) ? oa + width : -1;
-        const int64_t g = cur.row / p.rows_per_group;
-        s_grp[b * kSlots + slot_a] = g;
-        s_grp[b * kSlots + slot_a + 1] = g;
-      }
-      __syncwarp();
-      if (lane == 0) mbar_arrive(s_full + b);
-    }
-  } else {
-    reg_dealloc<kMelRegs>();
-    const int mw = warp - kWarps;
-    GroupMax gmax{p.stage == B200A_STAGE_FEAT ? p.group_max : nullptr, -1, -CUDART_INF_F};
-    int it = 0;
-    for (int64_t base = u0; base < p.total_units; base += stride, ++it) {
-      const int b = it & 1;
-      mbar_wait(s_full + b, (it >> 1) & 1);
+        prow_a[Ge::kNfft / 2] = pa[16];
+        prow_b[Ge::kNfft / 2] = pb[16];
+      }
+    }
+    if (l == 0) {
+      const int64_t ta = cur.ub * Ge::kFrames + 2 * gi;
+      const int64_t oa = (cur.row * p.frames + ta) * (int64_t)width + p.out_col0;
+      s_slot[slot_a] = (valid && ta < p.frames) ? oa : -1;
+      s_slot[slot_a + 1] = (valid && ta + 1 < p.frames) ? oa + width : -1;
+      const int64_t g = cur.row / p.rows_per_group;
+      s_grp[slot_a] = g;
+      s_grp[slot_a + 1] = g;
+    }
+    __syncthreads();
 #pragma unroll 1
-      for (int mt = 0; mt < kSlots / 16; ++mt)
-        contract_tile<kPitch>(p, s_plan, s_frags, frags_in_smem, mw, lane, s_pow + (size_t)(b * kSlots + 16 * mt) * kPitch,
-                              s_slot + b * kSlots + 16 * mt, s_grp + b * kSlots + 16 * mt, gmax);
-      __syncwarp();
-      if (lane == 0) mbar_arrive(s_empty + b);
-    }
-    gmax.flush();
-  }
+    for (int i = work_begin; i < work_end; ++i) {
+      const int w = s_plan->work[i], mt = w >> 8;
+      const int64_t* slot = s_slot + 16 * mt;
+      const int64_t* grp = s_grp + 16 * mt;
+      const int r = lane >> 2;
+      contract_item<kPitch>(p, s_plan->items[w & 255], s_frags, frags_in_smem, lane, s_pow + (size_t)16 * mt * kPitch,
+                            slot[r], slot[r + 8], grp[r], grp[r + 8], gmax);
+    }
+  }
+  gmax.flush();
 }
 
 constexpr int kEoN = 2048, kEoBins = 1025, kEoPitch = 1060, kEoSlots = 16;
@@ -1004,9 +1041,9 @@
 }
 
 template <int POWER_MODE, int G, int HG, bool KALDI>
-__global__ void __launch_bounds__((kWarps + kMelWarps) * 32, 1) stft_pow2_mel_kernel(const Pow2Params p) {
+__global__ void __launch_bounds__(kUniWarps * 32, 1) stft_pow2_mel_kernel(const Pow2Params p) {
   extern __shared__ __align__(128) unsigned char smem_raw[];
-  mel_body_mma<POWER_MODE, G, HG, kFftRegs, KALDI>(p, smem_raw);
+  mel_body<POWER_MODE, G, HG, KALDI>(p, smem_raw);
 }
 
 struct IstftPow2Params {
@@ -1027,18 +1064,17 @@
   constexpr int N = Ge::kNfft, NG = Ge::kGroups;
   extern __shared__ __align__(128) unsigned char smem_raw[];
   float2* s_tw = reinterpret_cast<float2*>(smem_raw);
-  float2* s_tile_all = s_tw + 32 * G;
+  float* s_win = reinterpret_cast<float*>(s_tw + 32 * G);
+  float2* s_tile_all = reinterpret_cast<float2*>(s_win + N);
   const int tid = threadIdx.x, lane = tid & 31, warp = tid >> 5;
   for (int i = tid; i < 32 * G; i += blockDim.x) s_tw[i] = p.tw2d[i];
+  {
+    const float gain = 1.f / ((float)N * p.hdr->scale);
+    for (int i = tid; i < N; i += blockDim.x) s_win[i] = p.window[i] * gain;
+  }
   __syncthreads();
   float2* grp_tile = s_tile_all + warp * Ge::kTileF2 + (lane / G) * Ge::kRegion;
   const int gi = lane / G, l = lane % G;
-  float wreg[32];
-  {
-    const float gain = 1.f / ((float)N * p.hdr->scale);
-#pragma unroll
-    for (int m = 0; m < 32; ++m) wreg[m] = p.window[l + G * m] * gain;
-  }
   UnitCursor cur;
   cur.init((int64_t)blockIdx.x * kIsWarps + warp, (int64_t)gridDim.x * kIsWarps, p.units_per_row);
   for (; cur.u < p.total_units; cur.advance()) {
@@ -1080,8 +1116,9 @@
     static_for<32>([&](auto mi) {
       constexpr int m = decltype(mi)::value;
       constexpr int slot = (m % NG) * G + m / NG;
-      if (has_a) fa[G * m] = a[slot].x * wreg[m];
-      if (has_b) fa[N + G * m] = -a[slot].y * wreg[m];
+      const float w = s_win[l + G * m];
+      if (has_a) fa[G * m] = a[slot].x * w;
+      if (has_b) fa[N + G * m] = -a[slot].y * w;
     });
   }
 }
@@ -1097,8 +1134,9 @@
 }
 
 __global__ void prepare_mma_kernel(const float* __restrict__ fb, const int2* __restrict__ bands, int n_bins, int n_mels,
-                                   int n_tiles, MelPlan* plan, float4* frags) {
-  __shared__ int t_kstart[kMaxItems], t_steps[kMaxItems];
+                                   int n_tiles, int n_mtiles, MelPlan* plan, float4* frags) {
+  __shared__ int t_kstart[kMaxItems], t_steps[kMaxItems], order[kMaxItems];
+  __shared__ unsigned char owner[kMaxMTiles * kMaxItems];
   if (threadIdx.x == 0) {
     int total = 0;
     for (int t = 0; t < n_tiles; ++t) {
@@ -1115,22 +1153,43 @@
     plan->n_tiles = n_tiles;
     plan->n_items = n_tiles;
     plan->total_steps = total;
-    plan->pad = 0;
-    int load[kWarps];
+    plan->n_work = n_mtiles * n_tiles;
+    int load[kUniWarps], cnt[kUniWarps];
     bool used[kMaxItems];
-    for (int w = 0; w < kWarps; ++w) { load[w] = 0; plan->warp_cnt[w] = 0; }
+    for (int w = 0; w < kMelWarps; ++w) { load[w] = 0; plan->warp_cnt[w] = 0; }
     for (int i = 0; i < n_tiles; ++i) used[i] = false;
     for (int k = 0; k < n_tiles; ++k) {
       int best = -1;
       for (int i = 0; i < n_tiles; ++i)
         if (!used[i] && (best < 0 || t_steps[i] > t_steps[best])) best = i;
       used[best] = true;
+      order[k] = best;
       int w = 0;
       for (int q = 1; q < kMelWarps; ++q)
         if (load[q] < load[w] || (load[q] == load[w] && plan->warp_cnt[q] < plan->warp_cnt[w])) w = q;
       plan->warp_items[w][plan->warp_cnt[w]++] = best;
       load[w] += t_steps[best] + 2;
     }
+    for (int w = 0; w < kUniWarps; ++w) { load[w] = 0; cnt[w] = 0; }
+    for (int k = 0; k < n_tiles; ++k)
+      for (int mt = 0; mt < n_mtiles; ++mt) {
+        int w = 0;
+        for (int q = 1; q < kUniWarps; ++q)
+          if (load[q] < load[w] || (load[q] == load[w] && cnt[q] < cnt[w])) w = q;
+        owner[k * n_mtiles + mt] = (unsigned char)w;
+        ++cnt[w];
+        load[w] += t_steps[order[k]] + 2;
+      }
+    int begin = 0;
+    for (int w = 0; w < kUniWarps; ++w) {
+      plan->work_begin[w] = begin;
+      begin += cnt[w];
+      cnt[w] = plan->work_begin[w];
+    }
+    for (int w = kUniWarps; w < kUniWarps + 4; ++w) plan->work_begin[w] = begin;
+    for (int k = 0; k < n_tiles; ++k)
+      for (int mt = 0; mt < n_mtiles; ++mt)
+        plan->work[cnt[owner[k * n_mtiles + mt]]++] = (unsigned short)((mt << 8) | order[k]);
   }
   __syncthreads();
   int off = 0;
@@ -1170,9 +1229,10 @@
   prepare_tw2d_kernel<<<(32 * G + 255) / 256, 256, 0, stream>>>(reinterpret_cast<float2*>(base + e.tw2d), G);
   if (d->n_fft == 2048) prepare_tw_eo_kernel<<<3, 256, 0, stream>>>(reinterpret_cast<float2*>(base + e.tw_eo));
   if (d->n_mels > 0 && mel_tiles(d->n_mels) <= kMaxItems) {
+    const int n_mtiles = d->n_fft == 2048 ? 0 : kUniWarps * 2 * (32 / G) / 16;
     prepare_mma_kernel<<<1, 256, 0, stream>>>(reinterpret_cast<const float*>(base + l.fb),
                                               reinterpret_cast<const int2*>(base + l.bands), d->n_fft / 2 + 1, d->n_mels,
-                                              mel_tiles(d->n_mels), reinterpret_cast<MelPlan*>(base + e.plan),
+                                              mel_tiles(d->n_mels), n_mtiles, reinterpret_cast<MelPlan*>(base + e.plan),
                                               reinterpret_cast<float4*>(base + e.frags));
   }
   return launch_status();
@@ -1192,7 +1252,7 @@
 static int launch_power(const Pow2Params& p, cudaStream_t stream) {
   using Ge = Geo<G>;
   constexpr int NW = 16;
-  const size_t smem = sizeof(float2) * (32 * 32 + NW * Ge::kTileF2) + sizeof(uint64_t) * NW;
+  const size_t smem = sizeof(float2) * (32 * 32 + NW * Ge::kTileF2) + sizeof(float) * Ge::kNfft + sizeof(uint64_t) * NW;
   auto kern = stft_pow2_power_kernel<POWER_MODE, G, HG, NW, false>;
   if constexpr (POWER_MODE != kComplexOut)
     if (p.kaldi) kern = stft_pow2_power_kernel<POWER_MODE, G, -1, NW, true>;
@@ -1208,17 +1268,16 @@
 static int launch_mel(const Pow2Params& p, cudaStream_t stream) {
   using Ge = Geo<G>;
   static_assert(sizeof(MelPlan) % 16 == 0, "fragment array must stay 16-byte aligned");
-  static_assert(Ge::kSlots <= kMaxSlots, "slot tables");
-  const size_t smem = sizeof(float2) * (32 * 32 + kWarps * Ge::kTileF2) + sizeof(float) * 2 * Ge::kSlots * Ge::kPitch +
-                      sizeof(int64_t) * 4 * Ge::kSlots + sizeof(uint64_t) * (kWarps + 4) + sizeof(MelPlan) +
-                      sizeof(float4) * 32 * kFragSmemSteps;
-  if (smem > 227 * 1024) return B200A_EUNSUPPORTED;
+  static_assert(Ge::kSlots <= kMaxSlots && Ge::kMTiles <= kMaxMTiles, "slot tables");
+  static_assert((Ge::kSlots * Ge::kPitch) % 4 == 0, "slot tables and plan stay 16-byte aligned");
+  constexpr size_t smem = mel_smem_bytes<G>();
+  static_assert(smem <= kSmemLimit, "16-warp mel kernel exceeds the shared-memory budget");
   auto kern = p.kaldi ? stft_pow2_mel_kernel<POWER_MODE, G, -1, true> : stft_pow2_mel_kernel<POWER_MODE, G, HG, false>;
-  if (cudaFuncSetAttribute(kern, cudaFuncAttributeMaxDynamicSharedMemorySize, 227 * 1024) != cudaSuccess)
+  if (cudaFuncSetAttribute(kern, cudaFuncAttributeMaxDynamicSharedMemorySize, kSmemLimit) != cudaSuccess)
     return B200A_ECUDA;
-  const int64_t grid = persistent_grid(p);
+  const int64_t grid = persistent_grid(p, kUniWarps);
   if (grid < 0) return B200A_ECUDA;
-  kern<<<(unsigned)grid, (kWarps + kMelWarps) * 32, smem, stream>>>(p);
+  kern<<<(unsigned)grid, kUniWarps * 32, smem, stream>>>(p);
   return launch_status();
 }
 
@@ -1305,8 +1364,12 @@
   p.db_mult = d->db_multiplier;
   p.db_amin = d->db_amin;
   p.db_offset = d->db_offset;
+  const bool mel = stage >= B200A_STAGE_MEL;
   const int half = d->center ? d->n_fft / 2 : 0;
-  const int stage_floats = 2 * (32 / G) * (32 * (G + 1) + (G == 8 ? 8 : 0));
+  const int stage_floats = !mel    ? 2 * (32 / G) * (32 * (G + 1) + (G == 8 ? 8 : 0))
+                           : G == 8  ? Geo<8>::kMelRegion
+                           : G == 16 ? Geo<16>::kMelRegion
+                                     : Geo<32>::kMelRegion;
   p.bulk_ok = d->hop % 4 == 0 && (half + d->pad) % 4 == 0 && row_stride % 4 == 0 &&
               (reinterpret_cast<uintptr_t>(wave) & 15) == 0 &&
               d->n_fft + (frames_per_unit - 1) * (int64_t)d->hop <= stage_floats;
@@ -1336,7 +1399,6 @@
   p.out_vec = (p.out_width % 4 == 0 && p.out_col0 % 4 == 0 && (reinterpret_cast<uintptr_t>(out) & 15) == 0)   ? 4
               : (p.out_width % 2 == 0 && p.out_col0 % 2 == 0 && (reinterpret_cast<uintptr_t>(out) & 7) == 0) ? 2
                                                                                                               : 1;
-  const bool mel = stage >= B200A_STAGE_MEL;
   if (eo) {
     p.bulk_ok = d->hop % 4 == 0 && (half + d->pad) % 4 == 0 && row_stride % 4 == 0 &&
                 (reinterpret_cast<uintptr_t>(wave) & 15) == 0;
@@ -1376,9 +1438,9 @@
     kern<<<grid, kIsWarps * 32, smem, stream>>>(p);
     return launch_status();
   };
-  if (G == 32) return launch(istft_pow2_kernel<32>, sizeof(float2) * (32 * 32 + kIsWarps * Geo<32>::kTileF2));
-  if (G == 16) return launch(istft_pow2_kernel<16>, sizeof(float2) * (32 * 16 + kIsWarps * Geo<16>::kTileF2));
-  return launch(istft_pow2_kernel<8>, sizeof(float2) * (32 * 8 + kIsWarps * Geo<8>::kTileF2));
-}
-
-}
+  if (G == 32) return launch(istft_pow2_kernel<32>, sizeof(float2) * (32 * 32 + kIsWarps * Geo<32>::kTileF2) + 4 * 1024);
+  if (G == 16) return launch(istft_pow2_kernel<16>, sizeof(float2) * (32 * 16 + kIsWarps * Geo<16>::kTileF2) + 4 * 512);
+  return launch(istft_pow2_kernel<8>, sizeof(float2) * (32 * 8 + kIsWarps * Geo<8>::kTileF2) + 4 * 256);
+}
+
+}
```
